# davidfang00/opticalflowdiffusion

Measured on NVIDIA B200. Metric: flows/sec DDIM-50 @436x1024, higher is better.
Workload: dtype bf16

## Files before the change

opticalflowdiffusion_b200/csrc/fd_conv_epi.cuh:

```cuda
#pragma once

#include "fd_tc.cuh"

namespace fdtc {

constexpr int kBlockM = 128;
constexpr int kEpiWarps = 8;
constexpr int kEpiThreads = kEpiWarps * 32;
constexpr int kSlabBytes = kBlockM * 128;

struct EpiTile {
  int img, h0, w0, n_tile;
};

struct EpiCtx {
  uint32_t tmem_base;
  uint32_t o_smem;
  uint32_t tfull0, tempty0;
  float* s_bias;
  float* s_stats;
  const CUtensorMap* map_out;
  const float* bias;
  const __nv_bfloat16* residual;
  double* gn_stats;
  int H, W, Cout, Wt;
  int shuffle_cq;
  float* head_out;
  const float* head_w;
  const float* head_b;
  int head_n, head_h0, head_w0, head_pt, head_pl;
  float* s_head;
  int phase;
  int dbg;
  int tempty_remote;
  const double* rt_stats;
  const float* rt_gamma;
  const float* rt_beta;
  float rt_eps;
  float* s_rt;
};

__device__ __forceinline__ float epi_silu_half(float h) {
  float t;
  asm("tanh.approx.f32 %0, %1;" : "=f"(t) : "f"(h));
  return fmaf(h, t, h);
}

__device__ __forceinline__ void mbar_arrive_cluster(uint32_t bar, uint32_t rank) {
  asm volatile(
      "{\n\t.reg .b32 ra;\n\t"
      "mapa.shared::cluster.u32 ra, %0, %1;\n\t"
      "mbarrier.arrive.shared::cluster.b64 _, [ra];\n\t}" ::"r"(bar),
      "r"(rank)
      : "memory");
}

template <int BLOCK_N, int GPT, int NBUF, int NACC = 2, class NextTile>
__device__ __forceinline__ void conv_epilogue(const EpiCtx& ec, NextTile next_tile) {
  constexpr int NCHUNK = BLOCK_N / 32;
  constexpr int CPW = NCHUNK / 2;
  constexpr int CPGT = GPT > 0 ? BLOCK_N / GPT : 32;
  constexpr int GIC = CPGT < 32 ? 32 / CPGT : 1;
  const int warp = threadIdx.x >> 5;
  const int lane = threadIdx.x & 31;
  const uint32_t tmem_base = ec.tmem_base;
  const uint32_t o_smem = ec.o_smem;
  float* const s_bias = ec.s_bias;
  float* const s_stats = ec.s_stats;
  {
    const int ew = warp - 2;
    const int et = threadIdx.x - 64;
    const int quarter = warp & 3;
    const int half = ew >> 2;
    const int row = quarter * 32 + lane;
    const int rr = row / ec.Wt, ww = row - rr * ec.Wt;
    float st_s[CPW > 0 ? CPW : 1][GIC], st_q[CPW > 0 ? CPW : 1][GIC];
#pragma unroll
    for (int a = 0; a < (CPW > 0 ? CPW : 1); ++a)
#pragma unroll
      for (int b = 0; b < GIC; ++b) st_s[a][b] = st_q[a][b] = 0.f;
    int st_img = -1, st_ntile = 0;
    int rt_img = -1, rt_ntile = -1;
    if (BLOCK_N == 64 && ec.head_out != nullptr) {
      for (int i = et; i < ec.head_n * 64; i += kEpiThreads) ec.s_head[i] = __ldg(ec.head_w + i);
    }
    uint32_t slab_count = 0;

    auto flush_stats = [&]() {
      if (GPT == 0 || st_img < 0) return;
      float* mine = s_stats + ew * 16;
      if (lane < 16) mine[lane] = 0.f;
      __syncwarp();
#pragma unroll
      for (int a = 0; a < (CPW > 0 ? CPW : 1); ++a)
#pragma unroll
        for (int b = 0; b < GIC; ++b) {
          const float s = fd_warp_sum(st_s[a][b]), q = fd_warp_sum(st_q[a][b]);
          if (lane == 0) {
            const int col = (2 * a + half) * 32 + b * CPGT;
            const int grp = col / CPGT;
            mine[grp * 2] += s;
            mine[grp * 2 + 1] += q;
          }
          st_s[a][b] = st_q[a][b] = 0.f;
        }
      named_bar_sync(2, kEpiThreads);
      if (et < 2 * GPT) {
        float sv = 0.f;
#pragma unroll
        for (int w8 = 0; w8 < kEpiWarps; ++w8) sv += s_stats[w8 * 16 + et];
        atomicAdd(ec.gn_stats + (long)st_img * 16 + st_ntile * 2 * GPT + et, (double)sv);
      }
      named_bar_sync(2, kEpiThreads);
    };

    EpiTile tc;
    for (int iter = 0; next_tile(iter, tc); ++iter) {
      const int as = iter % NACC;
      const uint32_t aphase = (iter / NACC) & 1;
      const int n_tile = tc.n_tile, img = tc.img, h0 = tc.h0, w0 = tc.w0;
      const int h = h0 + rr, w = w0 + ww;
      const bool valid = (h < ec.H) && (w < ec.W);
      const int n0 = n_tile * BLOCK_N;
      if (GPT > 0 && (img != st_img || n_tile != st_ntile)) {
        flush_stats();
        st_img = img;
        st_ntile = n_tile;
      }
      float* bias_s = s_bias + (as & 1) * BLOCK_N;
      for (int i = et; i < BLOCK_N; i += kEpiThreads) bias_s[i] = ec.bias ? __ldg(ec.bias + n0 + i) : 0.f;
      float* rt_s = ec.s_rt;
      if (ec.rt_stats != nullptr && (img != rt_img || n_tile != rt_ntile)) {
        rt_img = img;
        rt_ntile = n_tile;
        const int cpg = ec.Cout >> 3;
        const double cnt = (double)ec.H * (double)ec.W * (double)cpg;
        for (int i = et; i < BLOCK_N; i += kEpiThreads) {
          const int c = n0 + i;
          const int g = c / cpg;
          const double s = ec.rt_stats[((long)img * 8 + g) * 2], ss = ec.rt_stats[((long)img * 8 + g) * 2 + 1];
          const double mean = s / cnt;
          double var = ss / cnt - mean * mean;
          if (var < 0.0) var = 0.0;
          const float rstd = (float)(1.0 / sqrt(var + (double)ec.rt_eps));
          const float ga = __ldg(ec.rt_gamma + c) * rstd;
          rt_s[i] = 0.5f * ga;
          rt_s[BLOCK_N + i] = 0.5f * (__ldg(ec.rt_beta + c) - (float)mean * ga);
        }
      }

      const long pix = ((long)img * ec.H + h) * ec.W + w;
      const __nv_bfloat16* rrow = (ec.residual && valid) ? ec.residual + pix * ec.Cout + n0 : nullptr;
      uint4 rpre[4];
      if (rrow != nullptr) {
#pragma unroll
        for (int q = 0; q < 4; ++q) rpre[q] = __ldg(reinterpret_cast<const uint4*>(rrow + half * 32) + q);
      }
      mbar_wait(ec.tfull0 + 8u * as, aphase);
      tc_fence_after();
      if (ec.dbg & 8) {
        tc_fence_before();
        if (ec.tempty_remote) mbar_arrive_cluster(ec.tempty0 + 8u * as, 0);
        else mbar_arrive(ec.tempty0 + 8u * as);
        continue;
      }
#pragma unroll
      for (int slab = 0; slab < (BLOCK_N + 63) / 64; ++slab) {
        const uint32_t buf = o_smem + (slab_count % NBUF) * kSlabBytes;
        ++slab_count;
        if (ew == 0 && elect_one_sync()) tma_store_wait_read<NBUF - 1>();
        named_bar_sync(1, kEpiThreads);
        const int ci = slab * 2 + half;
        const int c = ci * 32;
        uint32_t acc[32];
        tmem_ld32(tmem_base + ((uint32_t)(quarter * 32) << 16) + (uint32_t)(as * BLOCK_N + c), acc);
        tmem_ld_wait();
        float v[32];
#pragma unroll
        for (int j4 = 0; j4 < 8; ++j4) {
          const float4 b4 = *reinterpret_cast<const float4*>(bias_s + c + j4 * 4);
          v[j4 * 4 + 0] = __uint_as_float(acc[j4 * 4 + 0]) + b4.x;
          v[j4 * 4 + 1] = __uint_as_float(acc[j4 * 4 + 1]) + b4.y;
          v[j4 * 4 + 2] = __uint_as_float(acc[j4 * 4 + 2]) + b4.z;
          v[j4 * 4 + 3] = __uint_as_float(acc[j4 * 4 + 3]) + b4.w;
        }
        if (rrow != nullptr) {
          uint4 rcur[4];
#pragma unroll
          for (int q = 0; q < 4; ++q) rcur[q] = rpre[q];
          if (slab + 1 < (BLOCK_N + 63) / 64) {
#pragma unroll
            for (int q = 0; q < 4; ++q) rpre[q] = __ldg(reinterpret_cast<const uint4*>(rrow + c + 64) + q);
          }
#pragma unroll
          for (int q = 0; q < 4; ++q) {
            const uint4 r4 = rcur[q];
            const uint32_t rw[4] = {r4.x, r4.y, r4.z, r4.w};
            if (ec.rt_stats != nullptr) {
              const float4 a0 = *reinterpret_cast<const float4*>(rt_s + c + q * 8), a1 = *reinterpret_cast<const float4*>(rt_s + c + q * 8 + 4);
              const float4 b0 = *reinterpret_cast<const float4*>(rt_s + BLOCK_N + c + q * 8),
                           b1 = *reinterpret_cast<const float4*>(rt_s + BLOCK_N + c + q * 8 + 4);
              const float aa[8] = {a0.x, a0.y, a0.z, a0.w, a1.x, a1.y, a1.z, a1.w};
              const float bb[8] = {b0.x, b0.y, b0.z, b0.w, b1.x, b1.y, b1.z, b1.w};
#pragma unroll
              for (int e = 0; e < 4; ++e) {
                const float2 f = fd_unpack_bf16(rw[e]);
                v[q * 8 + e * 2] += epi_silu_half(fmaf(aa[e * 2], f.x, bb[e * 2]));
                v[q * 8 + e * 2 + 1] += epi_silu_half(fmaf(aa[e * 2 + 1], f.y, bb[e * 2 + 1]));
              }
            } else {
#pragma unroll
              for (int e = 0; e < 4; ++e) {
                const float2 f = fd_unpack_bf16(rw[e]);
                v[q * 8 + e * 2] += f.x;
                v[q * 8 + e * 2 + 1] += f.y;
              }
            }
          }
        }
        if (GPT > 0 && valid) {
#pragma unroll
          for (int b = 0; b < GIC; ++b) {
            constexpr int span = CPGT < 32 ? CPGT : 32;
            float s = 0.f, q = 0.f;
#pragma unroll
            for (int j = 0; j < span; ++j) {
              const float x = v[b * span + j];
              s += x;
              q = fmaf(x, x, q);
            }
            st_s[slab][b] += s;
            st_q[slab][b] += q;
          }
        }
        if (BLOCK_N == 64 && ec.head_out != nullptr) {
          const float* hw = ec.s_head;
          float* hx = ec.s_head + 256 + (ew * 32 + lane) * 4;
          float d[4] = {0.f, 0.f, 0.f, 0.f};
#pragma unroll
          for (int o = 0; o < 4; ++o) {
            if (o < ec.head_n) {
#pragma unroll
              for (int j4 = 0; j4 < 8; ++j4) {
                const float4 w4 = *reinterpret_cast<const float4*>(hw + o * 64 + c + j4 * 4);
                d[o] = fmaf(v[j4 * 4 + 0], w4.x, d[o]);
                d[o] = fmaf(v[j4 * 4 + 1], w4.y, d[o]);
                d[o] = fmaf(v[j4 * 4 + 2], w4.z, d[o]);
                d[o] = fmaf(v[j4 * 4 + 3], w4.w, d[o]);
              }
            }
          }
          *reinterpret_cast<float4*>(hx) = make_float4(d[0], d[1], d[2], d[3]);
          tc_fence_before();
          if (ec.tempty_remote) mbar_arrive_cluster(ec.tempty0 + 8u * as, 0);
          else mbar_arrive(ec.tempty0 + 8u * as);
          named_bar_sync(1, kEpiThreads);
          if (half == 0 && valid) {
            const float4 o4 = *reinterpret_cast<const float4*>(ec.s_head + 256 + ((ew ^ 4) * 32 + lane) * 4);
            const float r4[4] = {d[0] + o4.x, d[1] + o4.y, d[2] + o4.z, d[3] + o4.w};
            const int hh = h - ec.head_pt, wq = w - ec.head_pl;
            if (hh >= 0 && hh < ec.head_h0 && wq >= 0 && wq < ec.head_w0) {
#pragma unroll
              for (int o = 0; o < 4; ++o)
                if (o < ec.head_n)
                  ec.head_out[(((long)img * ec.head_n + o) * ec.head_h0 + hh) * (long)ec.head_w0 + wq] = r4[o] + __ldg(ec.head_b + o);
            }
          }
          continue;
        }
        const uint32_t rbase = buf + (uint32_t)row * 128u;
#pragma unroll
        for (int q = 0; q < 4; ++q) {
          const uint32_t piece = (uint32_t)(half * 4 + q) ^ (uint32_t)(row & 7);
          const uint32_t o0 = fd_pack_bf16(v[q * 8 + 0], v[q * 8 + 1]), o1 = fd_pack_bf16(v[q * 8 + 2], v[q * 8 + 3]);
          const uint32_t o2 = fd_pack_bf16(v[q * 8 + 4], v[q * 8 + 5]), o3 = fd_pack_bf16(v[q * 8 + 6], v[q * 8 + 7]);
          asm volatile("st.shared.v4.b32 [%0], {%1, %2, %3, %4};" ::"r"(rbase + piece * 16u), "r"(o0), "r"(o1), "r"(o2),
                       "r"(o3)
                       : "memory");
        }
        fence_proxy_async_smem();
        if (slab == (BLOCK_N + 63) / 64 - 1) {
          tc_fence_before();
          if (ec.tempty_remote) mbar_arrive_cluster(ec.tempty0 + 8u * as, 0);
          else mbar_arrive(ec.tempty0 + 8u * as);
        }
        named_bar_sync(1, kEpiThreads);
        if (ew == 0 && elect_one_sync()) {
          const int cc = n0 + slab * 64;
          if (ec.shuffle_cq > 0) {
            const int pq = cc / ec.shuffle_cq;
            tma_store_5d(ec.map_out, buf, cc - pq * ec.shuffle_cq, pq & 1, w0, pq >> 1, h0);
          } else if (ec.phase >= 0) {
            tma_store_5d(ec.map_out, buf, cc, ec.phase & 1, w0, ec.phase >> 1, img * ec.H + h0);
          } else {
            tma_store_5d(ec.map_out, buf, cc, w0, h0, img, 0);
          }
          tma_store_commit();
        }
      }
    }
    flush_stats();
    __syncwarp();
    if (ew == 0 && elect_one_sync()) tma_store_wait_all();
  }
}

}
```

opticalflowdiffusion_b200/csrc/fd_conv_igemm.cu:

```cuda
#include "fd_conv_epi.cuh"

using namespace fdtc;

namespace {

constexpr int kBlockK = 64;
constexpr int kATileBytes = kBlockM * kBlockK * 2;
constexpr int kThreads = 64 + kEpiThreads + 32;

struct ConvParams {
  int N, H, W;
  int Cout;
  int KW;
  int taps;
  int pad_h, pad_w;
  int mode;
  int chunks0, chunks1;
  int R, Wt;
  int tiles_w, tiles_h, n_tiles, total_tiles;
  const float* bias;
  const __nv_bfloat16* residual;
  double* gn_stats;
  int shuffle_cq;
  int dbg;
  const double* rt_stats;
  const float* rt_gamma;
  const float* rt_beta;
  float rt_eps;
  int phase;
  float* head_out;
  const float* head_w;
  const float* head_b;
  int head_n, head_h0, head_w0, head_pt, head_pl;
};

template <int BLOCK_N, int SH = 0>
struct Cfg {
  static constexpr int kBTileBytes = BLOCK_N * kBlockK * 2;
  static constexpr int kStageBytes = kATileBytes + kBTileBytes;
  static constexpr int kStages = SH ? (BLOCK_N == 64 ? 6 : (BLOCK_N == 128 ? 5 : 3)) : (BLOCK_N == 64 ? 7 : (BLOCK_N == 128 ? 6 : 4));
  static constexpr int kStoreBufs = SH ? (BLOCK_N / 64 > 2 ? BLOCK_N / 64 : 2) : (BLOCK_N == 64 ? 2 : 1);
  static constexpr int kTmemCols = 2 * BLOCK_N;
  static constexpr int kHeadBytes = BLOCK_N == 64 ? (256 + kEpiWarps * 32 * 4) * 4 : 0;
  static constexpr int kTailBytes = 256  + 2 * BLOCK_N * 4  + kEpiWarps * 16 * 4  + 64 +
                                    4 * BLOCK_N * 4  + kHeadBytes;
  static constexpr int kSmemBytes = 1024 + kStages * kStageBytes + kStoreBufs * kSlabBytes + kTailBytes;
};

template <int BLOCK_N, int GPT, int SH>
__global__ void __launch_bounds__(kThreads, 1)
conv_igemm_kernel(const __grid_constant__ CUtensorMap map_a0, const __grid_constant__ CUtensorMap map_a1,
                  const __grid_constant__ CUtensorMap map_b, const __grid_constant__ CUtensorMap map_out,
                  const ConvParams p) {
  using C = Cfg<BLOCK_N, SH>;
  constexpr int STAGES = C::kStages;
  constexpr int NBUF = C::kStoreBufs;
  extern __shared__ uint8_t smem_raw[];
  const uint32_t base = (smem_u32(smem_raw) + 1023u) & ~1023u;
  uint8_t* gbase = smem_raw + (base - smem_u32(smem_raw));
  const uint32_t a_smem = base;
  const uint32_t b_smem = base + STAGES * kATileBytes;
  const uint32_t o_smem = base + STAGES * C::kStageBytes;
  const uint32_t bar_base = o_smem + NBUF * kSlabBytes;
  auto full_bar = [&](int s) { return bar_base + 8u * s; };
  auto empty_bar = [&](int s) { return bar_base + 8u * (STAGES + s); };
  auto tfull_bar = [&](int s) { return bar_base + 8u * (2 * STAGES + s); };
  auto tempty_bar = [&](int s) { return bar_base + 8u * (2 * STAGES + 2 + s); };
  uint8_t* gtail = gbase + STAGES * C::kStageBytes + NBUF * kSlabBytes + 256;
  float* s_bias = reinterpret_cast<float*>(gtail);
  float* s_stats = reinterpret_cast<float*>(gtail + 2 * BLOCK_N * 4);
  uint32_t* s_tmem = reinterpret_cast<uint32_t*>(gtail + 2 * BLOCK_N * 4 + kEpiWarps * 16 * 4);
  float* s_rt = reinterpret_cast<float*>(gtail + 2 * BLOCK_N * 4 + kEpiWarps * 16 * 4 + 64);
  float* s_head = s_rt + 4 * BLOCK_N;

  const int warp = threadIdx.x >> 5;
  const int lane = threadIdx.x & 31;
  const int cpt = p.chunks0 + p.chunks1;
  const int num_kb = p.taps * cpt;
  const int tiles_per_img = p.tiles_w * p.tiles_h;

  if (warp == 0 && lane == 0) {
    tma_prefetch_desc(&map_a0);
    tma_prefetch_desc(&map_a1);
    tma_prefetch_desc(&map_b);
    tma_prefetch_desc(&map_out);
    for (int s = 0; s < STAGES; ++s) {
      mbar_init(full_bar(s), 2);
      mbar_init(empty_bar(s), 1);
    }
    for (int s = 0; s < 2; ++s) {
      mbar_init(tfull_bar(s), 1);
      mbar_init(tempty_bar(s), kEpiThreads);
    }
    fence_barrier_init();
  }
  if (warp == 1) tmem_alloc(smem_u32(s_tmem), C::kTmemCols);
  tc_fence_before();
  __syncthreads();
  tc_fence_after();
  const uint32_t tmem_base = *s_tmem;

  if (warp == 0 || warp == 10) {
    if (elect_one_sync()) {
      int stage = opaque32(0);
      uint32_t phase = 0;
      const int tile0 = opaque32((int)blockIdx.x), tstep = opaque32((int)gridDim.x);
      if (warp == 0) {
        const bool skip = kDiag && (opaque32(p.dbg) & 1) != 0, mode0 = opaque32(p.mode) == 0;
        const int chunks0 = opaque32(p.chunks0), KW = opaque32(p.KW), cpt_ = opaque32(cpt), nkb = opaque32(num_kb);
        const uint64_t m0 = opaque64(reinterpret_cast<uint64_t>(&map_a0)), m1 = opaque64(reinterpret_cast<uint64_t>(&map_a1));
        for (int tile = tile0; tile < p.total_tiles; tile += tstep) {
          const int m_tile = tile / p.n_tiles;
          const int img = m_tile / tiles_per_img;
          const int rem = m_tile - img * tiles_per_img;
          const int th = rem / p.tiles_w;
          const int h0 = th * p.R;
          const int w0 = (rem - th * p.tiles_w) * p.Wt;
          const int bw = mode0 ? w0 - p.pad_w : 0, bh = mode0 ? h0 - p.pad_h : 0;
          int kx = 0, ky = 0, chunk = 0;
          for (int kb = 0; kb < nkb; ++kb) {
            const bool first = chunk < chunks0;
            const uint64_t ma = opaque64(first ? m0 : m1);
            const int c0 = opaque32((first ? chunk : chunk - chunks0) * kBlockK);
            const int c1 = opaque32(bw + kx);
            const int c2 = opaque32(mode0 ? bh + ky : w0);
            const int c3 = opaque32(mode0 ? img : ky);
            const int c4 = opaque32(mode0 ? 0 : h0);
            const uint32_t fb = (uint32_t)opaque32((int)full_bar(stage));
            const uint32_t dst = (uint32_t)opaque32((int)(a_smem + stage * kATileBytes));
            mbar_wait(empty_bar(stage), phase ^ 1u);
            if (skip) {
              mbar_arrive(fb);
            } else {
              mbar_expect_tx(fb, kATileBytes);
              tma_load_5d(dst, reinterpret_cast<const CUtensorMap*>(ma), fb, c0, c1, c2, c3, c4);
            }
            if (++stage == STAGES) { stage = 0; phase ^= 1u; }
            if (++chunk == cpt_) {
              chunk = 0;
              if (++kx == KW) { kx = 0; ++ky; }
            }
          }
        }
      } else {
        const bool skip = kDiag && (opaque32(p.dbg) & 2) != 0;
        const int nkb = opaque32(num_kb);
        const uint64_t mb = opaque64(reinterpret_cast<uint64_t>(&map_b));
        for (int tile = tile0; tile < p.total_tiles; tile += tstep) {
          const int n0 = (tile % p.n_tiles) * BLOCK_N;
          int k0 = 0;
          for (int kb = 0; kb < nkb; ++kb, k0 += kBlockK) {
            const uint32_t fb = (uint32_t)opaque32((int)full_bar(stage));
            const uint32_t dst = (uint32_t)opaque32((int)(b_smem + stage * C::kBTileBytes));
            const int ck = opaque32(k0), cn = opaque32(n0);
            mbar_wait(empty_bar(stage), phase ^ 1u);
            if (skip) {
              mbar_arrive(fb);
            } else {
              mbar_expect_tx(fb, C::kBTileBytes);
              tma_load_2d(dst, reinterpret_cast<const CUtensorMap*>(mb), fb, ck, cn);
            }
            if (++stage == STAGES) { stage = 0; phase ^= 1u; }
          }
        }
      }
    }
  } else if (warp == 1) {
    constexpr uint32_t idesc = umma_idesc_bf16(kBlockM, BLOCK_N);
    if (elect_one_sync()) {
      const uint64_t adesc0 = umma_desc_sw128(a_smem), bdesc0 = umma_desc_sw128(b_smem);
      int stage = 0;
      uint32_t phase = 0;
      int iter = 0;
      bool waited = false;
      const bool skip_mma = kDiag && (p.dbg & 4) != 0;
      uint64_t ad = opaque64(adesc0), bd = opaque64(bdesc0);
      for (int tile = blockIdx.x; tile < p.total_tiles; tile += gridDim.x, ++iter) {
        const int as = iter & 1;
        const uint32_t aphase = (iter >> 1) & 1;
        mbar_wait(tempty_bar(as), aphase ^ 1u);
        tc_fence_after();
        const uint32_t tmem_d = tmem_base + as * BLOCK_N;
        for (int kb = 0; kb < num_kb; ++kb) {
          if (!waited) mbar_wait(full_bar(stage), phase);
          tc_fence_after();
          if (!skip_mma) {
#pragma unroll
            for (int k = 0; k < kBlockK / 16; ++k) {
              umma_bf16(tmem_d, ad + (uint64_t)(2 * k), bd + (uint64_t)(2 * k), idesc, (kb | k) != 0 ? 1u : 0u);
            }
          }
          const uint32_t cur_empty = empty_bar(stage);
          if (++stage == STAGES) { stage = 0; phase ^= 1u; }
          ad = opaque64(adesc0 + (uint64_t)(stage * (kATileBytes >> 4)));
          bd = opaque64(bdesc0 + (uint64_t)(stage * (C::kBTileBytes >> 4)));
          waited = kb + 1 < num_kb;
          if (waited) mbar_wait(full_bar(stage), phase);
          umma_commit(cur_empty);
          if (kb == num_kb - 1) umma_commit(tfull_bar(as));
        }
      }
    }
    __syncwarp();
  } else if (warp >= 2 && warp < 2 + kEpiWarps) {
    EpiCtx ec;
    ec.tmem_base = tmem_base;
    ec.o_smem = o_smem;
    ec.tfull0 = tfull_bar(0);
    ec.tempty0 = tempty_bar(0);
    ec.s_bias = s_bias;
    ec.s_stats = s_stats;
    ec.map_out = &map_out;
    ec.bias = p.bias;
    ec.residual = p.residual;
    ec.gn_stats = p.gn_stats;
    ec.H = p.H; ec.W = p.W; ec.Cout = p.Cout; ec.Wt = p.Wt;
    ec.shuffle_cq = p.shuffle_cq;
    ec.tempty_remote = 0;
    ec.dbg = kDiag ? p.dbg : 0;
    ec.rt_stats = p.rt_stats; ec.rt_gamma = p.rt_gamma; ec.rt_beta = p.rt_beta; ec.rt_eps = p.rt_eps; ec.s_rt = s_rt;
    ec.phase = p.phase;
    ec.head_out = p.head_out; ec.head_w = p.head_w; ec.head_b = p.head_b; ec.head_n = p.head_n; ec.s_head = s_head;
    ec.head_h0 = p.head_h0; ec.head_w0 = p.head_w0; ec.head_pt = p.head_pt; ec.head_pl = p.head_pl;
    conv_epilogue<BLOCK_N, GPT, NBUF>(ec, [&](int iter, EpiTile& t) {
      const int tile = blockIdx.x + iter * gridDim.x;
      if (tile >= p.total_tiles) return false;
      t.n_tile = tile % p.n_tiles;
      const int m_tile = tile / p.n_tiles;
      t.img = m_tile / tiles_per_img;
      const int rem = m_tile - t.img * tiles_per_img;
      t.h0 = (rem / p.tiles_w) * p.R;
      t.w0 = (rem % p.tiles_w) * p.Wt;
      return true;
    });
  }

  tc_fence_before();
  __syncthreads();
  if (warp == 1) {
    tc_fence_after();
    tmem_dealloc(tmem_base, C::kTmemCols);
  }
}

constexpr uint32_t kPeerBitMask = 0xFEFFFFFFu;

__device__ __forceinline__ uint32_t cluster_ctarank() {
  uint32_t r;
  asm volatile("mov.u32 %0, %%cluster_ctarank;" : "=r"(r));
  return r;
}
__device__ __forceinline__ void cluster_sync_all() {
  asm volatile("barrier.cluster.arrive.release.aligned;" ::: "memory");
  asm volatile("barrier.cluster.wait.acquire.aligned;" ::: "memory");
}
__device__ __forceinline__ void tma2_load_5d(uint32_t dst, const CUtensorMap* m, uint32_t bar, int c0, int c1, int c2, int c3,
                                             int c4) {
  asm volatile(
      "cp.async.bulk.tensor.5d.cta_group::2.shared::cluster.global.mbarrier::complete_tx::bytes [%0], [%1, {%3, %4, %5, %6, %7}], [%2];" ::"r"(dst),
      "l"(m), "r"(bar & kPeerBitMask), "r"(c0), "r"(c1), "r"(c2), "r"(c3), "r"(c4)
      : "memory");
}
__device__ __forceinline__ void tma2_load_2d(uint32_t dst, const CUtensorMap* m, uint32_t bar, int c0, int c1) {
  asm volatile(
      "cp.async.bulk.tensor.2d.cta_group::2.shared::cluster.global.mbarrier::complete_tx::bytes [%0], [%1, {%3, %4}], [%2];" ::"r"(dst),
      "l"(m), "r"(bar & kPeerBitMask), "r"(c0), "r"(c1)
      : "memory");
}
__device__ __forceinline__ void umma2_bf16(uint32_t tmem_d, uint64_t adesc, uint64_t bdesc, uint32_t idesc, uint32_t accumulate) {
  asm volatile(
      "{\n\t.reg .pred p;\n\t"
      "setp.ne.b32 p, %4, 0;\n\t"
      "tcgen05.mma.cta_group::2.kind::f16 [%0], %1, %2, %3, p;\n\t}" ::"r"(tmem_d),
      "l"(adesc), "l"(bdesc), "r"(idesc), "r"(accumulate)
      : "memory");
}
__device__ __forceinline__ void umma2_commit(uint32_t bar) {
  asm volatile("tcgen05.commit.cta_group::2.mbarrier::arrive::one.shared::cluster.multicast::cluster.b64 [%0], %1;" ::"r"(bar),
               "h"((uint16_t)3)
               : "memory");
}

template <int BLOCK_N, int MT = 1>
struct PairCfg {
  static constexpr int kBHalfBytes = (BLOCK_N / 2) * kBlockK * 2;
  static constexpr int kStageBytes = MT * kATileBytes + kBHalfBytes;
  static constexpr int kStages = MT == 2 ? 5 : (BLOCK_N == 256 ? 5 : 7);
  static constexpr int kStoreBufs = MT == 2 ? 1 : 2;
  static constexpr int kAcc = 2 * MT;
  static constexpr int kTmemCols = kAcc * BLOCK_N;
  static constexpr int kTailBytes = 256 + 2 * BLOCK_N * 4 + kEpiWarps * 16 * 4 + 64 + 4 * BLOCK_N * 4;
  static constexpr int kSmemBytes = 1024 + kStages * kStageBytes + kStoreBufs * kSlabBytes + kTailBytes;
  static_assert(kTmemCols <= 512, "accumulators do not fit tensor memory");
};

template <int BLOCK_N, int GPT, int MT>
__global__ void __cluster_dims__(2, 1, 1) __launch_bounds__(kThreads, 1)
conv_igemm_pair_kernel(const __grid_constant__ CUtensorMap map_a0, const __grid_constant__ CUtensorMap map_a1,
                       const __grid_constant__ CUtensorMap map_b, const __grid_constant__ CUtensorMap map_out,
                       const ConvParams p) {
  using C = PairCfg<BLOCK_N, MT>;
  constexpr int STAGES = C::kStages;
  constexpr int NBUF = C::kStoreBufs;
  constexpr int NACC = C::kAcc;
  extern __shared__ uint8_t smem_raw[];
  const uint32_t base = (smem_u32(smem_raw) + 1023u) & ~1023u;
  uint8_t* gbase = smem_raw + (base - smem_u32(smem_raw));
  const uint32_t a_smem = base;
  const uint32_t b_smem = base + STAGES * MT * kATileBytes;
  const uint32_t o_smem = base + STAGES * C::kStageBytes;
  const uint32_t bar_base = o_smem + NBUF * kSlabBytes;
  auto full_bar = [&](int s) { return bar_base + 8u * s; };
  auto empty_bar = [&](int s) { return bar_base + 8u * (STAGES + s); };
  auto tfull_bar = [&](int s) { return bar_base + 8u * (2 * STAGES + s); };
  auto tempty_bar = [&](int s) { return bar_base + 8u * (2 * STAGES + NACC + s); };
  uint8_t* gtail = gbase + STAGES * C::kStageBytes + NBUF * kSlabBytes + 256;
  float* s_bias = reinterpret_cast<float*>(gtail);
  float* s_stats = reinterpret_cast<float*>(gtail + 2 * BLOCK_N * 4);
  uint32_t* s_tmem = reinterpret_cast<uint32_t*>(gtail + 2 * BLOCK_N * 4 + kEpiWarps * 16 * 4);
  float* s_rt = reinterpret_cast<float*>(gtail + 2 * BLOCK_N * 4 + kEpiWarps * 16 * 4 + 64);
  float* s_head = nullptr;

  const int warp = threadIdx.x >> 5;
  const int lane = threadIdx.x & 31;
  const uint32_t rank = cluster_ctarank();
  const int pair = blockIdx.x >> 1, npairs = gridDim.x >> 1;
  const int cpt = p.chunks0 + p.chunks1;
  const int num_kb = p.taps * cpt;
  const int tiles_per_img = p.tiles_w * p.tiles_h;
  const int super_tiles = p.total_tiles / (2 * MT);

  auto decode = [&](int st, int m, int& n_tile, int& img, int& h0, int& w0) {
    n_tile = st % p.n_tiles;
    const int m_tile = 2 * MT * (st / p.n_tiles) + (int)rank * MT + m;
    img = m_tile / tiles_per_img;
    const int rem = m_tile - img * tiles_per_img;
    h0 = (rem / p.tiles_w) * p.R;
    w0 = (rem % p.tiles_w) * p.Wt;
  };

  if (warp == 0 && lane == 0) {
    tma_prefetch_desc(&map_a0);
    tma_prefetch_desc(&map_a1);
    tma_prefetch_desc(&map_b);
    tma_prefetch_desc(&map_out);
    for (int s = 0; s < STAGES; ++s) {
      mbar_init(full_bar(s), 2);
      mbar_init(empty_bar(s), 1);
    }
    for (int s = 0; s < NACC; ++s) {
      mbar_init(tfull_bar(s), 1);
      mbar_init(tempty_bar(s), 2 * kEpiThreads);
    }
    fence_barrier_init();
  }
  if (warp == 1) {
    asm volatile("tcgen05.alloc.cta_group::2.sync.aligned.shared::cta.b32 [%0], %1;" ::"r"(smem_u32(s_tmem)), "r"(C::kTmemCols)
                 : "memory");
    asm volatile("tcgen05.relinquish_alloc_permit.cta_group::2.sync.aligned;" ::: "memory");
  }
  tc_fence_before();
  __syncthreads();
  cluster_sync_all();
  tc_fence_after();
  const uint32_t tmem_base = *s_tmem;

  if (warp == 0 || warp == 10) {
    if (elect_one_sync()) {
      int stage = opaque32(0);
      uint32_t phase = 0;
      const int st0 = opaque32(pair), ststep = opaque32(npairs), nkb = opaque32(num_kb);
      const bool leader = opaque32((int)rank) == 0;
      if (warp == 0) {
        const bool mode0 = opaque32(p.mode) == 0;
        const int chunks0 = opaque32(p.chunks0), KW = opaque32(p.KW), cpt_ = opaque32(cpt);
        const uint64_t m0 = opaque64(reinterpret_cast<uint64_t>(&map_a0)), m1 = opaque64(reinterpret_cast<uint64_t>(&map_a1));
        for (int st = st0; st < super_tiles; st += ststep) {
          int n_tile, img[MT], h0[MT], w0[MT], bw[MT], bh[MT];
#pragma unroll
          for (int m = 0; m < MT; ++m) {
            decode(st, m, n_tile, img[m], h0[m], w0[m]);
            bw[m] = mode0 ? w0[m] - p.pad_w : 0;
            bh[m] = mode0 ? h0[m] - p.pad_h : 0;
          }
          int kx = 0, ky = 0, chunk = 0;
          for (int kb = 0; kb < nkb; ++kb) {
            const bool first = chunk < chunks0;
            const uint64_t ma = opaque64(first ? m0 : m1);
            const int c0 = opaque32((first ? chunk : chunk - chunks0) * kBlockK);
            int c1[MT], c2[MT], c3[MT], c4[MT];
#pragma unroll
            for (int m = 0; m < MT; ++m) {
              c1[m] = opaque32(bw[m] + kx);
              c2[m] = opaque32(mode0 ? bh[m] + ky : w0[m]);
              c3[m] = opaque32(mode0 ? img[m] : ky);
              c4[m] = opaque32(mode0 ? 0 : h0[m]);
            }
            const uint32_t fb = (uint32_t)opaque32((int)full_bar(stage));
            const uint32_t dst = (uint32_t)opaque32((int)(a_smem + stage * MT * kATileBytes));
            mbar_wait(empty_bar(stage), phase ^ 1u);
            if (kDiag && (p.dbg & 1)) {
              if (leader) mbar_arrive(fb);
            } else {
              if (leader) mbar_expect_tx(fb, 2 * MT * kATileBytes);
#pragma unroll
              for (int m = 0; m < MT; ++m)
                tma2_load_5d(dst + m * kATileBytes, reinterpret_cast<const CUtensorMap*>(ma), fb, c0, c1[m], c2[m], c3[m], c4[m]);
            }
            if (++stage == STAGES) { stage = 0; phase ^= 1u; }
            if (++chunk == cpt_) {
              chunk = 0;
              if (++kx == KW) { kx = 0; ++ky; }
            }
          }
        }
      } else {
        const uint64_t mb = opaque64(reinterpret_cast<uint64_t>(&map_b));
        for (int st = st0; st < super_tiles; st += ststep) {
          const int n0 = (st % p.n_tiles) * BLOCK_N + (int)rank * (BLOCK_N / 2);
          int k0 = 0;
          for (int kb = 0; kb < nkb; ++kb, k0 += kBlockK) {
            const uint32_t fb = (uint32_t)opaque32((int)full_bar(stage));
            const uint32_t dst = (uint32_t)opaque32((int)(b_smem + stage * C::kBHalfBytes));
            const int ck = opaque32(k0), cn = opaque32(n0);
            mbar_wait(empty_bar(stage), phase ^ 1u);
            if (kDiag && (p.dbg & 2)) {
              if (leader) mbar_arrive(fb);
            } else {
              if (leader) mbar_expect_tx(fb, 2 * C::kBHalfBytes);
              tma2_load_2d(dst, reinterpret_cast<const CUtensorMap*>(mb), fb, ck, cn);
            }
            if (++stage == STAGES) { stage = 0; phase ^= 1u; }
          }
        }
      }
    }
  } else if (warp == 1) {
    if (rank == 0 && elect_one_sync()) {
      constexpr uint32_t idesc = umma_idesc_bf16(256, BLOCK_N);
      const uint64_t adesc0 = umma_desc_sw128(a_smem), bdesc0 = umma_desc_sw128(b_smem);
      int stage = 0;
      uint32_t phase = 0;
      int iter = 0;
      bool waited = false;
      uint64_t ad = opaque64(adesc0), bd = opaque64(bdesc0);
      for (int st = pair; st < super_tiles; st += npairs, ++iter) {
        const int as0 = (iter & 1) * MT;
        const uint32_t aphase = (iter >> 1) & 1;
#pragma unroll
        for (int m = 0; m < MT; ++m) mbar_wait(tempty_bar(as0 + m), aphase ^ 1u);
        tc_fence_after();
        const uint32_t tmem_d = tmem_base + as0 * BLOCK_N;
        for (int kb = 0; kb < num_kb; ++kb) {
          if (!waited) mbar_wait(full_bar(stage), phase);
          tc_fence_after();
#pragma unroll
          for (int m = 0; m < MT; ++m)
#pragma unroll
            for (int k = 0; k < kBlockK / 16; ++k)
              if (!(kDiag && (p.dbg & 4)))
                umma2_bf16(tmem_d + m * BLOCK_N, ad + (uint64_t)(m * (kATileBytes >> 4) + 2 * k), bd + (uint64_t)(2 * k), idesc,
                           (kb | k) != 0 ? 1u : 0u);
          const uint32_t cur_empty = empty_bar(stage);
          if (++stage == STAGES) { stage = 0; phase ^= 1u; }
          ad = opaque64(adesc0 + (uint64_t)(stage * (MT * kATileBytes >> 4)));
          bd = opaque64(bdesc0 + (uint64_t)(stage * (C::kBHalfBytes >> 4)));
          waited = kb + 1 < num_kb;
          if (waited) mbar_wait(full_bar(stage), phase);
          umma2_commit(cur_empty);
          if (kb == num_kb - 1) {
#pragma unroll
            for (int m = 0; m < MT; ++m) umma2_commit(tfull_bar(as0 + m));
          }
        }
      }
    }
    __syncwarp();
  } else if (warp >= 2 && warp < 2 + kEpiWarps) {
    EpiCtx ec;
    ec.tmem_base = tmem_base;
    ec.o_smem = o_smem;
    ec.tfull0 = tfull_bar(0);
    ec.tempty0 = tempty_bar(0);
    ec.s_bias = s_bias;
    ec.s_stats = s_stats;
    ec.map_out = &map_out;
    ec.bias = p.bias;
    ec.residual = p.residual;
    ec.gn_stats = p.gn_stats;
    ec.H = p.H; ec.W = p.W; ec.Cout = p.Cout; ec.Wt = p.Wt;
    ec.shuffle_cq = p.shuffle_cq;
    ec.tempty_remote = rank != 0;
    ec.dbg = kDiag ? p.dbg : 0;
    ec.rt_stats = p.rt_stats; ec.rt_gamma = p.rt_gamma; ec.rt_beta = p.rt_beta; ec.rt_eps = p.rt_eps; ec.s_rt = s_rt;
    ec.phase = p.phase;
    ec.head_out = p.head_out; ec.head_w = p.head_w; ec.head_b = p.head_b; ec.head_n = p.head_n; ec.s_head = s_head;
    ec.head_h0 = p.head_h0; ec.head_w0 = p.head_w0; ec.head_pt = p.head_pt; ec.head_pl = p.head_pl;
    conv_epilogue<BLOCK_N, GPT, NBUF, NACC>(ec, [&](int iter, EpiTile& t) {
      const int st = pair + (iter / MT) * npairs;
      if (st >= super_tiles) return false;
      decode(st, iter % MT, t.n_tile, t.img, t.h0, t.w0);
      return true;
    });
  }

  tc_fence_before();
  __syncthreads();
  cluster_sync_all();
  if (warp == 1) {
    tc_fence_after();
    asm volatile("tcgen05.dealloc.cta_group::2.sync.aligned.b32 %0, %1;" ::"r"(tmem_base), "r"(C::kTmemCols) : "memory");
  }
}

template <int BLOCK_N, int GPT, int MT = 1>
int launch_pair(const CUtensorMap& ma0, const CUtensorMap& ma1, const CUtensorMap& mb, const CUtensorMap& mo, const ConvParams& p,
                int sms, cudaStream_t st) {
  using C = PairCfg<BLOCK_N, MT>;
  static bool attr_set = false;
  if (!attr_set) {
    FD_CUDA(cudaFuncSetAttribute(conv_igemm_pair_kernel<BLOCK_N, GPT, MT>, cudaFuncAttributeMaxDynamicSharedMemorySize,
                                 C::kSmemBytes));
    attr_set = true;
  }
  const int units = p.total_tiles / MT;
  int grid = units < sms ? units : sms;
  grid &= ~1;
  conv_igemm_pair_kernel<BLOCK_N, GPT, MT><<<grid, kThreads, C::kSmemBytes, st>>>(ma0, ma1, mb, mo, p);
  FD_LAUNCH_CHECK();
  return FD_OK;
}

struct TileShape {
  int R, Wt;
};

TileShape pick_tile(int H, int W) {
  TileShape best{1, 128};
  long best_cost = -1;
  for (int wt = 128; wt >= 8; wt >>= 1) {
    const int r = 128 / wt;
    const long cost = (long)((W + wt - 1) / wt) * wt * (long)((H + r - 1) / r) * r;
    if (best_cost < 0 || cost < best_cost) {
      best_cost = cost;
      best = TileShape{r, wt};
    }
  }
  return best;
}

TileShape pick_tile_rows_divide(int H, int W) {
  TileShape best{1, 128};
  long best_cost = -1;
  for (int wt = 128; wt >= 8; wt >>= 1) {
    const int r = 128 / wt;
    if (H % r != 0) continue;
    const long cost = (long)((W + wt - 1) / wt) * wt * (long)H;
    if (best_cost < 0 || cost < best_cost) {
      best_cost = cost;
      best = TileShape{r, wt};
    }
  }
  return best;
}

template <int BLOCK_N, int GPT, int SH = 0>
int launch(const CUtensorMap& ma0, const CUtensorMap& ma1, const CUtensorMap& mb, const CUtensorMap& mo,
           const ConvParams& p, int sms, cudaStream_t st) {
  using C = Cfg<BLOCK_N, SH>;
  static bool attr_set = false;
  if (!attr_set) {
    FD_CUDA(cudaFuncSetAttribute(conv_igemm_kernel<BLOCK_N, GPT, SH>, cudaFuncAttributeMaxDynamicSharedMemorySize,
                                 C::kSmemBytes));
    attr_set = true;
  }
  const int grid = p.total_tiles < sms ? p.total_tiles : sms;
  conv_igemm_kernel<BLOCK_N, GPT, SH><<<grid, kThreads, C::kSmemBytes, st>>>(ma0, ma1, mb, mo, p);
  FD_LAUNCH_CHECK();
  return FD_OK;
}

}

int fd_conv3x3_strip_launch(const void* src0, int C0, const void* src1, int C1, const void* wpacked, const float* bias,
                            const void* residual,
                            void* out, double* gn_stats, int N, int H, int W, cudaStream_t st);

struct HeadArgs {
  float* out;
  const float* w;
  const float* b;
  int n, h0, w0, pt, pl;
};

static int conv_igemm_impl(const void* src0, int C0, const void* src1, int C1, const void* wpacked, const float* bias,
                           const void* residual, void* out, double* gn_stats, int N, int H, int W, int Cout, int KH, int KW,
                           int pad_h, int pad_w, int mode, int out_mode, const double* rt_stats, const float* rt_gamma,
                           const float* rt_beta, float rt_eps, void* stream, int phase = -1, const struct HeadArgs* head = nullptr);

extern "C" {

int fd_conv_igemm(const void* src0, int C0, const void* src1, int C1, const void* wpacked, const float* bias,
                  const void* residual, void* out, double* gn_stats, int N, int H, int W, int Cout, int KH, int KW,
                  int pad_h, int pad_w, int mode, void* stream) {
  return fd_conv_igemm_ex(src0, C0, src1, C1, wpacked, bias, residual, out, gn_stats, N, H, W, Cout, KH, KW, pad_h,
                          pad_w, mode, 0, stream);
}

int fd_conv_igemm_ex(const void* src0, int C0, const void* src1, int C1, const void* wpacked, const float* bias,
                     const void* residual, void* out, double* gn_stats, int N, int H, int W, int Cout, int KH, int KW,
                     int pad_h, int pad_w, int mode, int out_mode, void* stream) {
  return conv_igemm_impl(src0, C0, src1, C1, wpacked, bias, residual, out, gn_stats, N, H, W, Cout, KH, KW, pad_h, pad_w, mode,
                         out_mode, nullptr, nullptr, nullptr, 0.f, stream);
}

int fd_conv_igemm_rt(const void* src0, int C0, const void* src1, int C1, const void* wpacked, const float* bias,
                     const void* residual_raw, const double* res_stats, const float* res_gamma, const float* res_beta, float eps,
                     void* out, int N, int H, int W, int Cout, int KH, int KW, int pad_h, int pad_w, void* stream) {
  FD_REQUIRE(residual_raw && res_stats && res_gamma && res_beta, "conv_igemm_rt: null pointer");
  FD_REQUIRE(Cout % 64 == 0 && (Cout / 8) > 0, "conv_igemm_rt: Cout=%d", Cout);
  return conv_igemm_impl(src0, C0, src1, C1, wpacked, bias, residual_raw, out, nullptr, N, H, W, Cout, KH, KW, pad_h, pad_w, 0, 0,
                         res_stats, res_gamma, res_beta, eps, stream);
}

int fd_conv_igemm_rt_head(const void* src0, int C0, const void* src1, int C1, const void* wpacked, const float* bias,
                          const void* residual_raw, const double* res_stats, const float* res_gamma, const float* res_beta, float eps,
                          const float* head_w, const float* head_b, int head_n, float* out_nchw, int N, int H, int W, int H0, int W0,
                          int pad_top, int pad_left, void* stream) {
  FD_REQUIRE(residual_raw && res_stats && res_gamma && res_beta && head_w && head_b && out_nchw, "conv_igemm_rt_head: null pointer");
  FD_REQUIRE(head_n >= 1 && head_n <= 4, "conv_igemm_rt_head: head_n=%d (1..4)", head_n);
  FD_REQUIRE(H0 > 0 && W0 > 0 && pad_top >= 0 && pad_left >= 0 && pad_top + H0 <= H && pad_left + W0 <= W,
             "conv_igemm_rt_head: crop %dx%d at (%d, %d) outside %dx%d", H0, W0, pad_top, pad_left, H, W);
  const HeadArgs ha{out_nchw, head_w, head_b, head_n, H0, W0, pad_top, pad_left};
  return conv_igemm_impl(src0, C0, src1, C1, wpacked, bias, residual_raw, nullptr, nullptr, N, H, W, 64, 1, 1, 0, 0, 0, 0,
                         res_stats, res_gamma, res_beta, eps, stream, -1, &ha);
}

int fd_conv_igemm_up(const void* src, int Cin, const void* wpacked4, const float* bias, void* out, int N, int H, int W, int Cout,
                     void* stream) {
  FD_REQUIRE(src && wpacked4 && out, "conv_igemm_up: null pointer");
  FD_REQUIRE(Cin % 64 == 0 && Cout % 64 == 0, "conv_igemm_up: Cin=%d Cout=%d must be multiples of 64", Cin, Cout);
  const __nv_bfloat16* w4 = static_cast<const __nv_bfloat16*>(wpacked4);
  for (int ph = 0; ph < 4; ++ph) {
    const int a = ph >> 1, b = ph & 1;
    if (int e = conv_igemm_impl(src, Cin, nullptr, 0, w4 + (size_t)ph * Cout * 4 * Cin, bias, nullptr, out, nullptr, N, H, W, Cout, 2, 2,
                                1 - a, 1 - b, 0, 2, nullptr, nullptr, nullptr, 0.f, stream, ph))
      return e;
  }
  return FD_OK;
}

}

static int conv_igemm_impl(const void* src0, int C0, const void* src1, int C1, const void* wpacked, const float* bias,
                           const void* residual, void* out, double* gn_stats, int N, int H, int W, int Cout, int KH, int KW,
                           int pad_h, int pad_w, int mode, int out_mode, const double* rt_stats, const float* rt_gamma,
                           const float* rt_beta, float rt_eps, void* stream, int phase, const HeadArgs* head) {
  FD_REQUIRE(head == nullptr || (Cout == 64 && rt_stats != nullptr && out_mode == 0 && mode == 0 && gn_stats == nullptr && KH == 1 && KW == 1),
             "conv_igemm: the output head takes a 1x1 residual-transform conv with Cout = 64");
  if (head != nullptr && out == nullptr) out = const_cast<void*>(src0);
  FD_REQUIRE(out_mode == 0 || out_mode == 1 || out_mode == 2, "conv_igemm: out_mode %d", out_mode);
  FD_REQUIRE(out_mode != 2 || (mode == 0 && phase >= 0 && phase < 4 && residual == nullptr && gn_stats == nullptr && rt_stats == nullptr),
             "conv_igemm: the phase store takes a plain conv (no residual / statistics)");
  FD_REQUIRE(out_mode != 1 || (mode == 0 && KH == 1 && KW == 1 && pad_h == 0 && pad_w == 0 && C1 == 0 &&
                               residual == nullptr && gn_stats == nullptr && Cout % 256 == 0),
             "conv_igemm: the pixel-shuffle store is for 1x1 convs with Cout %% 256 == 0, no residual / statistics");
  FD_REQUIRE(src0 && wpacked && out, "conv_igemm: null pointer");
  FD_REQUIRE(N > 0 && H > 0 && W > 0, "conv_igemm: bad geometry N=%d H=%d W=%d", N, H, W);
  FD_REQUIRE(C0 > 0 && C0 % 64 == 0 && C1 >= 0 && C1 % 64 == 0, "conv_igemm: C0=%d C1=%d must be multiples of 64", C0, C1);
  FD_REQUIRE(src1 != nullptr || C1 == 0, "conv_igemm: C1 > 0 needs src1");
  FD_REQUIRE(Cout > 0 && Cout % 64 == 0, "conv_igemm: Cout=%d must be a multiple of 64", Cout);
  FD_REQUIRE(mode == 0 || mode == 1, "conv_igemm: mode %d", mode);
  FD_REQUIRE(mode == 0 || (C1 == 0 && gn_stats == nullptr), "conv_igemm: mode 1 takes one source and no statistics");
  FD_REQUIRE(KH >= 1 && KW >= 1 && KH * KW <= 64, "conv_igemm: bad kernel %dx%d", KH, KW);
  {
    const bool chans_ok = (C0 == 64 && (C1 == 0 || C1 == 64)) || (C0 == 128 && C1 == 0);
    if (mode == 0 && KH == 3 && KW == 3 && pad_h == 1 && pad_w == 1 && chans_ok && Cout == 64 && W >= 128 && out_mode == 0 &&
        rt_stats == nullptr)
      return fd_conv3x3_strip_launch(src0, C0, src1, C1, wpacked, bias, residual, out, gn_stats, N, H, W, (cudaStream_t)stream);
  }
  static int sms = 0;
  if (sms == 0) {
    int dev = 0;
    FD_CUDA(cudaGetDevice(&dev));
    FD_CUDA(cudaDeviceGetAttribute(&sms, cudaDevAttrMultiProcessorCount, dev));
  }
  ConvParams p{};
  p.Cout = Cout;
  p.mode = mode;
  p.chunks0 = C0 / 64;
  p.chunks1 = C1 / 64;
  p.bias = bias;
  p.residual = static_cast<const __nv_bfloat16*>(residual);
  p.gn_stats = gn_stats;
  p.rt_stats = rt_stats; p.rt_gamma = rt_gamma; p.rt_beta = rt_beta; p.rt_eps = rt_eps;
  p.phase = out_mode == 2 ? phase : -1;
  if (head != nullptr) {
    p.head_out = head->out; p.head_w = head->w; p.head_b = head->b; p.head_n = head->n;
    p.head_h0 = head->h0; p.head_w0 = head->w0; p.head_pt = head->pt; p.head_pl = head->pl;
  }
  CUtensorMap ma0, ma1, mb, mo;
  TileShape ts;
  if (mode == 0) {
    int n = N, h = H, w = W;
    if (out_mode == 1) {
      n = 1;
      h = N * H;
    } else if (KH == 1 && KW == 1 && pad_h == 0 && pad_w == 0 && gn_stats == nullptr && rt_stats == nullptr) {
      FD_REQUIRE((long)N * H * W < (1L << 31), "conv_igemm: too many pixels");
      w = N * H * W;
      h = 1;
      n = 1;
    }
    p.N = n; p.H = h; p.W = w;
    p.KW = KW;
    p.taps = KH * KW;
    p.pad_h = pad_h;
    p.pad_w = pad_w;
    ts = out_mode == 2 ? pick_tile_rows_divide(h, w) : pick_tile(h, w);
    const uint32_t box[5] = {64, (uint32_t)ts.Wt, (uint32_t)ts.R, 1, 1};
    {
      const uint64_t dims[5] = {(uint64_t)C0, (uint64_t)w, (uint64_t)h, (uint64_t)n, 1};
      const uint64_t str[4] = {(uint64_t)C0 * 2, (uint64_t)w * C0 * 2, (uint64_t)h * w * C0 * 2, (uint64_t)n * h * w * C0 * 2};
      if (int e = make_tmap_bf16(&ma0, src0, 5, dims, str, box)) return e;
    }
    if (C1 > 0) {
      const uint64_t dims[5] = {(uint64_t)C1, (uint64_t)w, (uint64_t)h, (uint64_t)n, 1};
      const uint64_t str[4] = {(uint64_t)C1 * 2, (uint64_t)w * C1 * 2, (uint64_t)h * w * C1 * 2, (uint64_t)n * h * w * C1 * 2};
      if (int e = make_tmap_bf16(&ma1, src1, 5, dims, str, box)) return e;
    } else {
      ma1 = ma0;
    }
  } else {
    p.N = 1; p.H = N * H; p.W = W;
    p.KW = 2;
    p.taps = 4;
    ts = pick_tile(p.H, p.W);
    const uint64_t dims[5] = {(uint64_t)C0, 2, (uint64_t)W, 2, (uint64_t)N * H};
    const uint64_t str[4] = {(uint64_t)C0 * 2, (uint64_t)2 * C0 * 2, (uint64_t)2 * W * C0 * 2, (uint64_t)4 * W * C0 * 2};
    const uint32_t box[5] = {64, 1, (uint32_t)ts.Wt, 1, (uint32_t)ts.R};
    if (int e = make_tmap_bf16(&ma0, src0, 5, dims, str, box)) return e;
    ma1 = ma0;
  }
  p.R = ts.R;
  p.Wt = ts.Wt;
  p.tiles_w = (p.W + ts.Wt - 1) / ts.Wt;
  p.tiles_h = (p.H + ts.R - 1) / ts.R;
  const int block_n = (Cout % 256 == 0) ? 256 : ((Cout % 128 == 0) ? 128 : 64);
  p.n_tiles = Cout / block_n;
  const long total = (long)p.N * p.tiles_w * p.tiles_h * p.n_tiles;
  FD_REQUIRE(total < (1L << 31), "conv_igemm: too many tiles");
  p.total_tiles = (int)total;
  const bool stats_ = gn_stats != nullptr;
  const bool store_heavy_ = !stats_ && p.taps * (p.chunks0 + p.chunks1) <= 4;
  static const int dbg = fd_diag_bits("FD_CONV_DBG");
  p.dbg = dbg;
  const bool use_pair = block_n >= 128 && !store_heavy_ && out_mode != 1 && ((long)p.N * p.tiles_w * p.tiles_h) % 2 == 0 &&
                        p.total_tiles >= 2;
  {
    const uint64_t K = (uint64_t)p.taps * (C0 + C1);
    const uint64_t dims[2] = {K, (uint64_t)Cout};
    const uint64_t str[1] = {K * 2};
    const uint32_t box[2] = {64, (uint32_t)(use_pair ? block_n / 2 : block_n)};
    if (int e = make_tmap_bf16(&mb, wpacked, 2, dims, str, box)) return e;
  }
  if (out_mode == 1) {
    const uint64_t cq = (uint64_t)Cout / 4;
    p.shuffle_cq = (int)cq;
    const uint64_t dims[5] = {cq, 2, (uint64_t)p.W, 2, (uint64_t)p.H};
    const uint64_t str[4] = {cq * 2, 2 * cq * 2, (uint64_t)2 * p.W * cq * 2, (uint64_t)4 * p.W * cq * 2};
    const uint32_t box[5] = {64, 1, (uint32_t)ts.Wt, 1, (uint32_t)ts.R};
    if (int e = make_tmap_bf16(&mo, out, 5, dims, str, box)) return e;
  } else if (out_mode == 2) {
    const uint64_t c = (uint64_t)Cout;
    const uint64_t dims[5] = {c, 2, (uint64_t)p.W, 2, (uint64_t)p.N * p.H};
    const uint64_t str[4] = {c * 2, 2 * c * 2, (uint64_t)2 * p.W * c * 2, (uint64_t)4 * p.W * c * 2};
    const uint32_t box[5] = {64, 1, (uint32_t)ts.Wt, 1, (uint32_t)ts.R};
    if (int e = make_tmap_bf16(&mo, out, 5, dims, str, box)) return e;
  } else {
    const uint64_t dims[5] = {(uint64_t)Cout, (uint64_t)p.W, (uint64_t)p.H, (uint64_t)p.N, 1};
    const uint64_t str[4] = {(uint64_t)Cout * 2, (uint64_t)p.W * Cout * 2, (uint64_t)p.H * p.W * Cout * 2,
                             (uint64_t)p.N * p.H * p.W * Cout * 2};
    const uint32_t box[5] = {64, (uint32_t)ts.Wt, (uint32_t)ts.R, 1, 1};
    if (int e = make_tmap_bf16(&mo, out, 5, dims, str, box)) return e;
  }
  cudaStream_t st = (cudaStream_t)stream;
  const bool stats = gn_stats != nullptr;
  if (stats) FD_REQUIRE(p.n_tiles == 1 || p.n_tiles == 2, "conv_igemm: statistics need Cout in {64,128,256,512}");
  const bool store_heavy = !stats && p.taps * (p.chunks0 + p.chunks1) <= 4;
  if (store_heavy) {
    if (block_n == 256) return launch<256, 0, 1>(ma0, ma1, mb, mo, p, sms, st);
    if (block_n == 128) return launch<128, 0, 1>(ma0, ma1, mb, mo, p, sms, st);
    return launch<64, 0, 1>(ma0, ma1, mb, mo, p, sms, st);
  }
  if (use_pair && block_n == 256) {
    if (!stats) return launch_pair<256, 0>(ma0, ma1, mb, mo, p, sms, st);
    return p.n_tiles == 1 ? launch_pair<256, 8>(ma0, ma1, mb, mo, p, sms, st) : launch_pair<256, 4>(ma0, ma1, mb, mo, p, sms, st);
  }
  if (use_pair) {
    const bool mt2 = ((long)p.N * p.tiles_w * p.tiles_h) % 4 == 0 && p.total_tiles >= 4;
    if (mt2) return stats ? launch_pair<128, 8, 2>(ma0, ma1, mb, mo, p, sms, st) : launch_pair<128, 0, 2>(ma0, ma1, mb, mo, p, sms, st);
    return stats ? launch_pair<128, 8>(ma0, ma1, mb, mo, p, sms, st) : launch_pair<128, 0>(ma0, ma1, mb, mo, p, sms, st);
  }
  if (block_n == 256) {
    if (!stats) return launch<256, 0>(ma0, ma1, mb, mo, p, sms, st);
    return p.n_tiles == 1 ? launch<256, 8>(ma0, ma1, mb, mo, p, sms, st) : launch<256, 4>(ma0, ma1, mb, mo, p, sms, st);
  }
  if (block_n == 128) return stats ? launch<128, 8>(ma0, ma1, mb, mo, p, sms, st) : launch<128, 0>(ma0, ma1, mb, mo, p, sms, st);
  return stats ? launch<64, 8>(ma0, ma1, mb, mo, p, sms, st) : launch<64, 0>(ma0, ma1, mb, mo, p, sms, st);
}
```

opticalflowdiffusion_b200/csrc/fd_conv_strip.cu:

```cuda
#include "fd_conv_epi.cuh"

using namespace fdtc;

namespace {

constexpr int kC = 64;
constexpr int kTileW = 128;
constexpr int kStripPx = kTileW + 2;
constexpr int kStripTx = kStripPx * 128;
constexpr int kStripBytes = 136 * 128;
constexpr int kNS = 5;
constexpr int kWTapBytes = kC * kC * 2;
constexpr int kWBytes = 9 * kWTapBytes;
constexpr int kThreads = 64 + kEpiThreads + 64;
constexpr int kTail = 256 + 2 * kC * 4 + kEpiWarps * 16 * 4 + 64;
constexpr int kSmemBytes = 1024 + kWBytes + kNS * kStripBytes + 2 * kSlabBytes + kTail;

__device__ __forceinline__ void utccp_128x256b(uint32_t tmem_dst, uint64_t sdesc) {
  asm volatile("tcgen05.cp.cta_group::1.128x256b [%0], %1;" ::"r"(tmem_dst), "l"(sdesc) : "memory");
}
__device__ __forceinline__ void umma_ts_bf16(uint32_t tmem_d, uint32_t tmem_a, uint64_t bdesc, uint32_t idesc, uint32_t accumulate) {
  asm volatile(
      "{\n\t.reg .pred p;\n\t"
      "setp.ne.b32 p, %4, 0;\n\t"
      "tcgen05.mma.cta_group::1.kind::f16 [%0], [%1], %2, %3, p;\n\t}" ::"r"(tmem_d),
      "r"(tmem_a), "l"(bdesc), "r"(idesc), "r"(accumulate)
      : "memory");
}
constexpr int kATmemCol0 = 2 * kC;
constexpr int kATmemSlotCols = 3 * (kC / 2);
constexpr int kATmemSlots = 4;

__device__ __forceinline__ float silu_tanh(float z) {
  const float h = 0.5f * z;
  float t;
  asm("tanh.approx.f32 %0, %1;" : "=f"(t) : "f"(h));
  return fmaf(h, t, h);
}

struct StripParams {
  int N, H, W;
  int wblocks, total_rows;
  int tile_w;
  int c_off;
  int w_k0, w_kstride;
  const float* bias;
  const __nv_bfloat16* residual;
  double* gn_stats;
  const double* in_stats;
  const float* in_gamma;
  const float* in_beta;
  const float* in_ss;
  long in_ss_stride;
  float in_eps;
  int dbg;
};

struct StripWalk {
  int cur, end;
  __device__ __forceinline__ explicit StripWalk(const StripParams& p) {
    cur = (int)((long)p.total_rows * blockIdx.x / gridDim.x);
    end = (int)((long)p.total_rows * (blockIdx.x + 1) / gridDim.x);
  }
  __device__ __forceinline__ bool next(const StripParams& p, int& n, int& w0, int& ra, int& rb) {
    if (cur >= end) return false;
    const int col = cur / p.H;
    ra = cur - col * p.H;
    const int rows = min(p.H - ra, end - cur);
    rb = ra + rows;
    n = col / p.wblocks;
    w0 = (col - n * p.wblocks) * p.tile_w;
    cur += rows;
    return true;
  }
};

template <int GPT, class NextTile>
__device__ __forceinline__ void strip_epilogue2(const EpiCtx& ec, NextTile next_tile) {
  const int warp = threadIdx.x >> 5, lane = threadIdx.x & 31;
  const int ew = warp - 2;
  const int quarter = warp & 3, group = ew >> 2;
  const int gt = (ew & 3) * 32 + lane;
  const int row = quarter * 32 + lane;
  const int bar_id = 1 + group;
  float* const bias_s = ec.s_bias + group * kC;
  float* const s_stats = ec.s_stats + group * 64;
  constexpr int NG = GPT > 0 ? GPT : 1;
  constexpr int CPG = kC / 8;
  float st_s[NG], st_q[NG];
#pragma unroll
  for (int b = 0; b < NG; ++b) st_s[b] = st_q[b] = 0.f;
  int st_img = -1;
  const uint32_t buf = ec.o_smem + group * kSlabBytes;
  if (gt < kC) bias_s[gt] = ec.bias ? __ldg(ec.bias + gt) : 0.f;
  named_bar_sync(bar_id, 128);

  auto flush_stats = [&]() {
    if (GPT == 0 || st_img < 0) return;
    float* mine = s_stats + (ew & 3) * 16;
#pragma unroll
    for (int b = 0; b < NG; ++b) {
      const float s = fd_warp_sum(st_s[b]), q = fd_warp_sum(st_q[b]);
      if (lane == 0) {
        mine[b * 2] = s;
        mine[b * 2 + 1] = q;
      }
      st_s[b] = st_q[b] = 0.f;
    }
    named_bar_sync(bar_id, 128);
    if (gt < 2 * GPT) {
      const float sv = (s_stats[gt] + s_stats[16 + gt]) + (s_stats[32 + gt] + s_stats[48 + gt]);
      atomicAdd(ec.gn_stats + (long)st_img * 16 + gt, (double)sv);
    }
    named_bar_sync(bar_id, 128);
  };

  EpiTile tc;
  for (int iter = 0; next_tile(iter, tc); ++iter) {
    if ((iter & 1) != group) continue;
    const int as = group;
    const uint32_t aphase = (iter >> 1) & 1;
    const int img = tc.img, h = tc.h0, w0 = tc.w0;
    const int w = w0 + row;
    const bool valid = w < ec.W;
    if (GPT > 0 && img != st_img) {
      flush_stats();
      st_img = img;
    }
    mbar_wait(ec.tfull0 + 8u * as, aphase);
    tc_fence_after();
    if (kDiag && (ec.dbg & 8)) {
      tc_fence_before();
      mbar_arrive(ec.tempty0 + 8u * as);
      continue;
    }
    uint32_t acc[2][32];
    const uint32_t taddr = ec.tmem_base + ((uint32_t)(quarter * 32) << 16) + (uint32_t)(as * kC);
    tmem_ld32(taddr, acc[0]);
    tmem_ld32(taddr + 32, acc[1]);
    tmem_ld_wait();
    tc_fence_before();
    mbar_arrive(ec.tempty0 + 8u * as);
    const long pix = ((long)img * ec.H + h) * ec.W + w;
    uint32_t packed[32];
#pragma unroll
    for (int hc = 0; hc < 2; ++hc) {
      float v[32];
#pragma unroll
      for (int j4 = 0; j4 < 8; ++j4) {
        const float4 b4 = *reinterpret_cast<const float4*>(bias_s + hc * 32 + j4 * 4);
        v[j4 * 4 + 0] = __uint_as_float(acc[hc][j4 * 4 + 0]) + b4.x;
        v[j4 * 4 + 1] = __uint_as_float(acc[hc][j4 * 4 + 1]) + b4.y;
        v[j4 * 4 + 2] = __uint_as_float(acc[hc][j4 * 4 + 2]) + b4.z;
        v[j4 * 4 + 3] = __uint_as_float(acc[hc][j4 * 4 + 3]) + b4.w;
      }
      if (ec.residual != nullptr && valid) {
        const __nv_bfloat16* rrow = ec.residual + pix * kC + hc * 32;
#pragma unroll
        for (int q = 0; q < 4; ++q) {
          const uint4 r4 = __ldg(reinterpret_cast<const uint4*>(rrow) + q);
          const uint32_t rw[4] = {r4.x, r4.y, r4.z, r4.w};
#pragma unroll
          for (int e = 0; e < 4; ++e) {
            const float2 f = fd_unpack_bf16(rw[e]);
            v[q * 8 + e * 2] += f.x;
            v[q * 8 + e * 2 + 1] += f.y;
          }
        }
      }
      if (GPT > 0 && valid) {
#pragma unroll
        for (int b = 0; b < 4; ++b) {
          float s = 0.f, q = 0.f;
#pragma unroll
          for (int j = 0; j < CPG; ++j) {
            const float x = v[b * CPG + j];
            s += x;
            q = fmaf(x, x, q);
          }
          st_s[(hc * 4 + b) % NG] += s;
          st_q[(hc * 4 + b) % NG] += q;
        }
      }
#pragma unroll
      for (int j = 0; j < 16; ++j) packed[hc * 16 + j] = fd_pack_bf16(v[2 * j], v[2 * j + 1]);
    }
    if ((ew & 3) == 0 && elect_one_sync()) tma_store_wait_read<0>();
    named_bar_sync(bar_id, 128);
    const uint32_t rbase = buf + (uint32_t)row * 128u;
#pragma unroll
    for (int q = 0; q < 8; ++q) {
      const uint32_t piece = (uint32_t)q ^ (uint32_t)(row & 7);
      asm volatile("st.shared.v4.b32 [%0], {%1, %2, %3, %4};" ::"r"(rbase + piece * 16u), "r"(packed[q * 4]),
                   "r"(packed[q * 4 + 1]), "r"(packed[q * 4 + 2]), "r"(packed[q * 4 + 3])
                   : "memory");
    }
    fence_proxy_async_smem();
    named_bar_sync(bar_id, 128);
    if ((ew & 3) == 0 && elect_one_sync()) {
      tma_store_5d(ec.map_out, buf, 0, w0, h, img, 0);
      tma_store_commit();
    }
  }
  flush_stats();
  __syncwarp();
  if ((ew & 3) == 0 && elect_one_sync()) tma_store_wait_all();
}

template <int GPT>
__global__ void __launch_bounds__(kThreads, 1)
conv3x3_strip_kernel(const __grid_constant__ CUtensorMap map_in, const __grid_constant__ CUtensorMap map_w,
                     const __grid_constant__ CUtensorMap map_out, const StripParams p) {
  extern __shared__ uint8_t smem_raw[];
  const uint32_t base = (smem_u32(smem_raw) + 1023u) & ~1023u;
  uint8_t* gbase = smem_raw + (base - smem_u32(smem_raw));
  const uint32_t w_smem = base;
  const uint32_t s_smem = base + kWBytes;
  const uint32_t o_smem = s_smem + kNS * kStripBytes;
  const uint32_t bar_base = o_smem + 2 * kSlabBytes;
  const uint32_t wfull_bar = bar_base;
  auto full_bar = [&](int s) { return bar_base + 8u * (1 + s); };
  auto empty_bar = [&](int s) { return bar_base + 8u * (1 + kNS + s); };
  auto tfull_bar = [&](int s) { return bar_base + 8u * (1 + 2 * kNS + s); };
  auto tempty_bar = [&](int s) { return bar_base + 8u * (3 + 2 * kNS + s); };
  auto xfull_bar = [&](int s) { return bar_base + 8u * (5 + 2 * kNS + s); };
  const bool fuse_in = p.in_stats != nullptr;
  uint8_t* gtail = gbase + kWBytes + kNS * kStripBytes + 2 * kSlabBytes + 256;
  float* s_bias = reinterpret_cast<float*>(gtail);
  float* s_stats = reinterpret_cast<float*>(gtail + 2 * kC * 4);
  uint32_t* s_tmem = reinterpret_cast<uint32_t*>(gtail + 2 * kC * 4 + kEpiWarps * 16 * 4);
  const int warp = threadIdx.x >> 5, lane = threadIdx.x & 31;

  if (warp == 0 && lane == 0) {
    tma_prefetch_desc(&map_in);
    tma_prefetch_desc(&map_w);
    tma_prefetch_desc(&map_out);
    mbar_init(wfull_bar, 1);
    for (int s = 0; s < kNS; ++s) {
      mbar_init(full_bar(s), 1);
      mbar_init(empty_bar(s), 1);
      mbar_init(xfull_bar(s), 64);
    }
    for (int s = 0; s < 2; ++s) {
      mbar_init(tfull_bar(s), 1);
      mbar_init(tempty_bar(s), 128);
    }
    fence_barrier_init();
  }
  constexpr uint32_t kTmemCols = 512;
  if (warp == 1) tmem_alloc(smem_u32(s_tmem), kTmemCols);
  tc_fence_before();
  __syncthreads();
  tc_fence_after();
  const uint32_t tmem_base = *s_tmem;

  if (warp == 0) {
    if (elect_one_sync()) {
      mbar_expect_tx(wfull_bar, kWBytes);
      for (int tap = 0; tap < 9; ++tap)
        tma_load_2d(w_smem + tap * kWTapBytes, &map_w, wfull_bar, tap * p.w_kstride + p.w_k0, 0);
      uint32_t seq = 0;
      StripWalk walk(p);
      int n, w0, ra, rb;
      while (walk.next(p, n, w0, ra, rb)) {
        for (int y = ra - 1; y <= rb; ++y, ++seq) {
          const int slot = seq % kNS;
          const uint32_t phase = (seq / kNS) & 1u;
          mbar_wait(empty_bar(slot), phase ^ 1u);
          mbar_expect_tx(full_bar(slot), kStripTx);
          tma_load_5d(s_smem + slot * kStripBytes, &map_in, full_bar(slot), p.c_off, w0 - 1, y, n, 0);
        }
      }
    }
  } else if (warp == 1) {
    if (elect_one_sync()) {
      constexpr uint32_t idesc = umma_idesc_bf16(kBlockM, kC);
      mbar_wait(wfull_bar, 0);
      tc_fence_after();
      const uint64_t bdesc0 = umma_desc_sw128(w_smem);
      const uint32_t a_tmem0 = tmem_base + kATmemCol0;
      StripWalk cwalk(p);
      int c_left = 0;
      uint32_t cseq = 0;
      auto ready_bar = [&](uint32_t slot) { return fuse_in ? xfull_bar(slot) : full_bar(slot); };
      auto copy_strip = [&]() {
        const uint32_t slot = cseq % kNS;
        mbar_wait(ready_bar(slot), (cseq / kNS) & 1u);
        tc_fence_after();
        const uint32_t dst = a_tmem0 + (cseq % kATmemSlots) * kATmemSlotCols;
        const uint64_t sd = umma_desc_sw128(s_smem + slot * kStripBytes);
#pragma unroll
        for (int kx = 0; kx < 3; ++kx)
#pragma unroll
          for (int k = 0; k < kC / 16; ++k)
            if (!(kDiag && (p.dbg & 64)))
            utccp_128x256b(dst + kx * (kC / 2) + k * 8, sd + (uint64_t)(kx * 8 + 2 * k));
        umma_commit(empty_bar(slot));
        ++cseq;
      };
      auto strips_left = [&]() {
        while (c_left == 0) {
          int cn, cw0, cra, crb;
          if (!cwalk.next(p, cn, cw0, cra, crb)) return false;
          c_left = crb - cra + 2;
        }
        return true;
      };
      struct Claim {
        bool more, inter;
        uint32_t slot, phase, dst;
        uint64_t sd;
      };
      auto claim = [&](uint32_t f) {
        Claim c{};
        c.more = cseq < f + 4 && strips_left();
        if (c.more) {
          c.slot = cseq % kNS;
          c.phase = (cseq / kNS) & 1u;
          c.dst = a_tmem0 + (cseq % kATmemSlots) * kATmemSlotCols;
          c.sd = umma_desc_sw128(s_smem + c.slot * kStripBytes);
          ++cseq;
          --c_left;
        }
        return c;
      };
      auto landed = [&](Claim& c) { c.inter = c.more && mbar_try_wait(ready_bar(c.slot), c.phase); };
      long long dg_t0 = 0, dg_mma = 0, dg_tail = 0;
      unsigned long long dg_ns0 = 0;
      if (kDiag) {
        dg_t0 = clock64();
        asm volatile("mov.u64 %0, %%globaltimer;" : "=l"(dg_ns0));
      }
      StripWalk walk(p);
      int wn, ww0, wra, wrb;
      int iter = 0;
      if (walk.next(p, wn, ww0, wra, wrb)) {
        int rows = wrb - wra, j = 0;
        uint32_t f = 0;
        while (cseq < f + 3) {
          strips_left();
          copy_strip();
          --c_left;
        }
        mbar_wait(tempty_bar(0), 1u);
        Claim cp = claim(f);
        landed(cp);
        tc_fence_after();
        while (true) {
          const int as = iter & 1;
          const uint32_t tmem_d = tmem_base + as * kC;
          bool has_next = false, boundary = false;
          uint32_t f_next = 0;
          Claim cp_next{};
          long long dg_m = 0;
          if (kDiag) dg_m = clock64();
#pragma unroll
          for (int ky = 0; ky < 3; ++ky) {
            const uint32_t a_strip = a_tmem0 + ((f + ky) % kATmemSlots) * kATmemSlotCols;
#pragma unroll
            for (int kx = 0; kx < 3; ++kx) {
              const uint64_t bdesc = bdesc0 + (uint64_t)((ky * 3 + kx) * (kWTapBytes >> 4));
#pragma unroll
              for (int k = 0; k < kC / 16; ++k) {
                if (!(kDiag && (p.dbg & 4)))
                  umma_ts_bf16(tmem_d, a_strip + kx * (kC / 2) + k * 8, bdesc + (uint64_t)(2 * k), idesc, (ky | kx | k) != 0 ? 1u : 0u);
                const int m = (ky * 3 + kx) * 4 + k;
                if (m % 3 == 2 && cp.inter && !(kDiag && (p.dbg & 64))) {
                  const int c = m / 3, ckx = c >> 2, ck = c & 3;
                  utccp_128x256b(cp.dst + ckx * (kC / 2) + ck * 8, cp.sd + (uint64_t)(ckx * 8 + 2 * ck));
                }
                if (m == 5) {
                  if (j + 1 < rows) {
                    has_next = true;
                    f_next = f + 1;
                  } else if (walk.next(p, wn, ww0, wra, wrb)) {
                    has_next = boundary = true;
                    f_next = f + 3;
                  }
                }
                if (m == 14 && has_next && !boundary) cp_next = claim(f_next);
                if (m == 23 && has_next && !boundary) mbar_wait(tempty_bar((iter + 1) & 1), (((iter + 1) >> 1) & 1) ^ 1u);
                if (m == 32 && has_next && !boundary) landed(cp_next);
              }
            }
          }
          umma_commit(tfull_bar(as));
          if (kDiag) { dg_mma += clock64() - dg_m; dg_m = clock64(); }
          if (cp.inter) {
            umma_commit(empty_bar(cp.slot));
          } else if (cp.more) {
            mbar_wait(ready_bar(cp.slot), cp.phase);
            tc_fence_after();
#pragma unroll
            for (int c = 0; c < 12; ++c)
              if (!(kDiag && (p.dbg & 64))) utccp_128x256b(cp.dst + (c >> 2) * (kC / 2) + (c & 3) * 8, cp.sd + (uint64_t)((c >> 2) * 8 + 2 * (c & 3)));
            umma_commit(empty_bar(cp.slot));
          }
          if (!has_next) break;
          if (boundary) {
            rows = wrb - wra;
            j = 0;
            while (cseq < f_next + 3) {
              strips_left();
              copy_strip();
              --c_left;
            }
            mbar_wait(tempty_bar((iter + 1) & 1), (((iter + 1) >> 1) & 1) ^ 1u);
            cp_next = claim(f_next);
            landed(cp_next);
          } else {
            ++j;
          }
          tc_fence_after();
          f = f_next;
          cp = cp_next;
          ++iter;
          if (kDiag) dg_tail += clock64() - dg_m;
        }
        ++iter;
      }
      if (kDiag && (p.dbg & 128) && (blockIdx.x == 0 || blockIdx.x == 77)) {
        unsigned long long ns1;
        asm volatile("mov.u64 %0, %%globaltimer;" : "=l"(ns1));
        const long long cyc = clock64() - dg_t0;
        printf("strip TS issuer block %d: %d tiles, %lld cycles (%.0f / tile): MMA stream %lld, between tiles %lld, %llu ns -> %.2f GHz\n",
               blockIdx.x, iter, cyc, (double)cyc / iter, dg_mma, dg_tail, ns1 - dg_ns0, (double)cyc / (double)(ns1 - dg_ns0));
      }
    }
    __syncwarp();
  } else if (warp == 10 || warp == 11) {
    if (fuse_in) {
      const int tl = (warp - 10) * 32 + lane;
      const int q = tl & 7, r0 = tl >> 3;
      float a[8], b[8];
      int cur_n = -1;
      uint32_t seq = 0;
      StripWalk walk(p);
      int n, w0, ra, rb;
      while (walk.next(p, n, w0, ra, rb)) {
        if (n != cur_n) {
          cur_n = n;
          const int C = kC, cpg = C >> 3;
          const double cnt = (double)p.H * (double)p.W * cpg;
          const int g = (q * 8) / cpg;
          const double sm = p.in_stats[((long)n * 8 + g) * 2], ss = p.in_stats[((long)n * 8 + g) * 2 + 1];
          const double mean = sm / cnt;
          double var = ss / cnt - mean * mean;
          if (var < 0.0) var = 0.0;
          const float rstd = (float)(1.0 / sqrt(var + (double)p.in_eps));
#pragma unroll
          for (int j = 0; j < 8; ++j) {
            const int c = q * 8 + j;
            float ga = __ldg(p.in_gamma + c) * rstd;
            float be = __ldg(p.in_beta + c) - (float)mean * ga;
            if (p.in_ss != nullptr) {
              const float sc = __ldg(p.in_ss + (long)n * p.in_ss_stride + c) + 1.f;
              const float sh = __ldg(p.in_ss + (long)n * p.in_ss_stride + C + c);
              ga *= sc;
              be = be * sc + sh;
            }
            a[j] = 0.5f * ga;
            b[j] = 0.5f * be;
          }
        }
        for (int y = ra - 1; y <= rb; ++y, ++seq) {
          const uint32_t slot = seq % kNS;
          mbar_wait(full_bar(slot), (seq / kNS) & 1u);
          if (y >= 0 && y < p.H) {
            const int rlo = w0 > 0 ? 0 : 1 - w0;
            const int rhi = min(kStripPx, p.W - w0 + 1);
            int r = r0 < rlo ? r0 + (((rlo - r0) + 7) & ~7) : r0;
            uint8_t* gp8 = gbase + kWBytes + slot * kStripBytes + r * 128 + ((q ^ r0) << 4);
#pragma unroll 4
            for (; r < rhi; r += 8, gp8 += 1024) {
              uint4* gp = reinterpret_cast<uint4*>(gp8);
              const uint4 v = *gp;
              const uint32_t xw[4] = {v.x, v.y, v.z, v.w};
              float o[8];
#pragma unroll
              for (int e = 0; e < 4; ++e) {
                const float h0 = fmaf(a[2 * e], __uint_as_float(xw[e] << 16), b[2 * e]);
                const float h1 = fmaf(a[2 * e + 1], __uint_as_float(xw[e] & 0xffff0000u), b[2 * e + 1]);
                float t0, t1;
                asm("tanh.approx.f32 %0, %1;" : "=f"(t0) : "f"(h0));
                asm("tanh.approx.f32 %0, %1;" : "=f"(t1) : "f"(h1));
                o[2 * e] = fmaf(h0, t0, h0);
                o[2 * e + 1] = fmaf(h1, t1, h1);
              }
              uint4 w4;
              w4.x = fd_pack_bf16(o[0], o[1]);
              w4.y = fd_pack_bf16(o[2], o[3]);
              w4.z = fd_pack_bf16(o[4], o[5]);
              w4.w = fd_pack_bf16(o[6], o[7]);
              *gp = w4;
            }
          }
          fence_proxy_async_smem();
          mbar_arrive(xfull_bar(slot));
        }
      }
    }
  } else if (warp >= 2 && warp < 2 + kEpiWarps) {
    EpiCtx ec;
    ec.tmem_base = tmem_base;
    ec.o_smem = o_smem;
    ec.tfull0 = tfull_bar(0);
    ec.tempty0 = tempty_bar(0);
    ec.s_bias = s_bias;
    ec.s_stats = s_stats;
    ec.map_out = &map_out;
    ec.bias = p.bias;
    ec.residual = p.residual;
    ec.gn_stats = p.gn_stats;
    ec.H = p.H; ec.W = p.W; ec.Cout = kC; ec.Wt = kTileW;
    ec.shuffle_cq = 0;
    ec.tempty_remote = 0;
    ec.dbg = kDiag ? p.dbg : 0;
    ec.rt_stats = nullptr; ec.rt_gamma = nullptr; ec.rt_beta = nullptr; ec.rt_eps = 0.f; ec.s_rt = nullptr;
    ec.phase = -1;
    ec.head_out = nullptr; ec.head_w = nullptr; ec.head_b = nullptr; ec.head_n = 0; ec.s_head = nullptr;
    ec.head_h0 = ec.head_w0 = ec.head_pt = ec.head_pl = 0;
    StripWalk walk(p);
    int j = 0, n = 0, w0 = 0, ra = 0, rb = 0;
    auto next = [&](int, EpiTile& t) {
      while (ra + j >= rb) {
        if (!walk.next(p, n, w0, ra, rb)) return false;
        j = 0;
      }
      t.img = n;
      t.h0 = ra + j;
      t.w0 = w0;
      t.n_tile = 0;
      ++j;
      return true;
    };
    strip_epilogue2<GPT>(ec, next);
  }

  tc_fence_before();
  __syncthreads();
  if (warp == 1) {
    tc_fence_after();
    tmem_dealloc(tmem_base, kTmemCols);
  }
}

}

struct StripInputNorm {
  const double* stats;
  const float *gamma, *beta, *scale_shift;
  long ss_stride;
  float eps;
};

static int strip_launch(const void* src0, int C0, const void* src1, int C1, const void* wpacked, const float* bias,
                        const void* residual, void* out, double* gn_stats, int N, int H, int W, const StripInputNorm& in,
                        cudaStream_t st);

int fd_conv3x3_strip_launch(const void* src0, int C0, const void* src1, int C1, const void* wpacked, const float* bias,
                            const void* residual, void* out, double* gn_stats, int N, int H, int W, cudaStream_t st) {
  return strip_launch(src0, C0, src1, C1, wpacked, bias, residual, out, gn_stats, N, H, W, StripInputNorm{}, st);
}

extern "C" int fd_conv3x3_gnsilu_in(const void* src, const double* in_stats, const float* in_gamma, const float* in_beta,
                                    const float* in_scale_shift, long in_ss_stride, float in_eps, const void* wpacked,
                                    const float* bias, const void* residual, void* out, double* gn_stats, int N, int H, int W,
                                    void* stream) {
  FD_REQUIRE(src && in_stats && in_gamma && in_beta && wpacked && out && N > 0 && H > 0 && W >= 64,
             "conv3x3_gnsilu_in: bad argument (needs 64 -> 64 channels, W >= 64)");
  StripInputNorm in{in_stats, in_gamma, in_beta, in_scale_shift, in_ss_stride, in_eps};
  return strip_launch(src, 64, nullptr, 0, wpacked, bias, residual, out, gn_stats, N, H, W, in, (cudaStream_t)stream);
}

static int strip_launch(const void* src0, int C0, const void* src1, int C1, const void* wpacked, const float* bias,
                        const void* residual, void* out, double* gn_stats, int N, int H, int W, const StripInputNorm& in,
                        cudaStream_t st) {
  static int sms = 0;
  if (sms == 0) {
    int dev = 0;
    FD_CUDA(cudaGetDevice(&dev));
    FD_CUDA(cudaDeviceGetAttribute(&sms, cudaDevAttrMultiProcessorCount, dev));
  }
  const int cin = C0 + C1;
  const int passes = cin / 64;
  StripParams p{};
  p.N = N; p.H = H; p.W = W;
  p.tile_w = kTileW;
  p.wblocks = (W + p.tile_w - 1) / p.tile_w;
  p.total_rows = N * p.wblocks * H;
  p.w_kstride = cin;
  CUtensorMap mw, mo;
  {
    const uint64_t dO[5] = {(uint64_t)kC, (uint64_t)W, (uint64_t)H, (uint64_t)N, 1};
    const uint64_t sO[4] = {(uint64_t)kC * 2, (uint64_t)W * kC * 2, (uint64_t)H * W * kC * 2, (uint64_t)N * H * W * kC * 2};
    const uint32_t box_out[5] = {64, (uint32_t)p.tile_w, 1, 1, 1};
    if (int e = make_tmap_bf16(&mo, out, 5, dO, sO, box_out)) return e;
    const uint64_t K = (uint64_t)9 * cin;
    const uint64_t dims[2] = {K, (uint64_t)kC};
    const uint64_t str[1] = {K * 2};
    const uint32_t box[2] = {64, 64};
    if (int e = make_tmap_bf16(&mw, wpacked, 2, dims, str, box)) return e;
  }
  const int grid = p.total_rows < sms ? p.total_rows : sms;
  static bool attr_set = false;
  if (!attr_set) {
    FD_CUDA(cudaFuncSetAttribute(conv3x3_strip_kernel<8>, cudaFuncAttributeMaxDynamicSharedMemorySize, kSmemBytes));
    FD_CUDA(cudaFuncSetAttribute(conv3x3_strip_kernel<0>, cudaFuncAttributeMaxDynamicSharedMemorySize, kSmemBytes));
    attr_set = true;
  }
  p.in_stats = in.stats;
  p.in_gamma = in.gamma;
  p.in_beta = in.beta;
  p.in_ss = in.scale_shift;
  p.in_ss_stride = in.ss_stride;
  p.in_eps = in.eps;
  static const int dbg = fd_diag_bits("FD_CONV_DBG");
  p.dbg = dbg;
  for (int pass = 0; pass < passes; ++pass) {
    const bool last = pass == passes - 1;
    const bool from1 = pass == 1 && C1 > 0;
    const void* src = from1 ? src1 : src0;
    const int csrc = from1 ? C1 : C0;
    CUtensorMap mi;
    const uint64_t d[5] = {(uint64_t)csrc, (uint64_t)W, (uint64_t)H, (uint64_t)N, 1};
    const uint64_t sB[4] = {(uint64_t)csrc * 2, (uint64_t)W * csrc * 2, (uint64_t)H * W * csrc * 2, (uint64_t)N * H * W * csrc * 2};
    const uint32_t box_in[5] = {64, (uint32_t)kStripPx, 1, 1, 1};
    if (int e = make_tmap_bf16(&mi, src, 5, d, sB, box_in)) return e;
    p.c_off = (pass == 1 && C1 == 0) ? 64 : 0;
    p.w_k0 = pass * 64;
    p.bias = last ? bias : nullptr;
    p.residual = static_cast<const __nv_bfloat16*>(pass > 0 ? out : residual);
    p.gn_stats = last ? gn_stats : nullptr;
    if (p.gn_stats != nullptr) conv3x3_strip_kernel<8><<<grid, kThreads, kSmemBytes, st>>>(mi, mw, mo, p);
    else conv3x3_strip_kernel<0><<<grid, kThreads, kSmemBytes, st>>>(mi, mw, mo, p);
    FD_LAUNCH_CHECK();
  }
  return FD_OK;
}
```

Baseline: 9.216.

## Prefetch conv residual tiles into a shared-memory ring via TMA

Residual tensors added in the conv epilogues were previously read per thread with __ldg (with a one-slab register prefetch). They are now loaded by TMA into a small mbarrier-guarded shared-memory ring that is issued ahead across tiles, in both the igemm/pair kernels and the strip conv kernel. The aim is to take global residual latency off the epilogue's critical path. Bias reloads are also skipped when the n-tile is unchanged, and the head bias is cached in shared memory. The cost is extra shared memory, which drops one pipeline stage for some configs, plus more barriers and more complexity.

```diff
diff --git a/opticalflowdiffusion_b200/csrc/fd_conv_epi.cuh b/opticalflowdiffusion_b200/csrc/fd_conv_epi.cuh
--- a/opticalflowdiffusion_b200/csrc/fd_conv_epi.cuh
+++ b/opticalflowdiffusion_b200/csrc/fd_conv_epi.cuh
@@ -22,6 +22,9 @@
   const CUtensorMap* map_out;
   const float* bias;
   const __nv_bfloat16* residual;
+  const CUtensorMap* map_res;
+  uint32_t r_smem;
+  uint32_t rfull0;
   double* gn_stats;
   int H, W, Cout, Wt;
   int shuffle_cq;
@@ -55,8 +58,11 @@
       : "memory");
 }
 
-template <int BLOCK_N, int GPT, int NBUF, int NACC = 2, class NextTile>
+template <int BLOCK_N, int GPT, int NBUF, int NACC = 2, int RS = 0, class NextTile>
 __device__ __forceinline__ void conv_epilogue(const EpiCtx& ec, NextTile next_tile) {
+  static_assert(RS == 0 || RS >= 2, "a one-slot residual ring is no deeper than the register prefetch");
+  constexpr int NSLAB = (BLOCK_N + 63) / 64;
+  constexpr uint32_t kRS = RS > 0 ? RS : 1;
   constexpr int NCHUNK = BLOCK_N / 32;
   constexpr int CPW = NCHUNK / 2;
   constexpr int CPGT = GPT > 0 ? BLOCK_N / GPT : 32;
@@ -81,10 +87,24 @@
       for (int b = 0; b < GIC; ++b) st_s[a][b] = st_q[a][b] = 0.f;
     int st_img = -1, st_ntile = 0;
     int rt_img = -1, rt_ntile = -1;
+    int bias_nt0 = -1, bias_nt1 = -1;
     if (BLOCK_N == 64 && ec.head_out != nullptr) {
       for (int i = et; i < ec.head_n * 64; i += kEpiThreads) ec.s_head[i] = __ldg(ec.head_w + i);
+      if (et < ec.head_n) ec.s_head[256 + kEpiThreads * 4 + et] = __ldg(ec.head_b + et);
     }
     uint32_t slab_count = 0;
+    const bool rtma = RS > 0 && ec.residual != nullptr;
+    auto res_issue = [&](uint32_t s) {
+      EpiTile t;
+      if (!next_tile((int)(s / NSLAB), t)) return;
+      const uint32_t slot = s % kRS;
+      const uint32_t bar = ec.rfull0 + 8u * slot;
+      mbar_expect_tx(bar, kSlabBytes);
+      tma_load_5d(ec.r_smem + slot * kSlabBytes, ec.map_res, bar, t.n_tile * BLOCK_N + (int)(s % NSLAB) * 64, t.w0, t.h0,
+                  t.img, 0);
+    };
+    if (rtma && ew == 0 && elect_one_sync())
+      for (int s = 0; s < RS; ++s) res_issue((uint32_t)s);
 
     auto flush_stats = [&]() {
       if (GPT == 0 || st_img < 0) return;
@@ -128,7 +148,11 @@
         st_ntile = n_tile;
       }
       float* bias_s = s_bias + (as & 1) * BLOCK_N;
-      for (int i = et; i < BLOCK_N; i += kEpiThreads) bias_s[i] = ec.bias ? __ldg(ec.bias + n0 + i) : 0.f;
+      if (((as & 1) ? bias_nt1 : bias_nt0) != n_tile) {
+        if (as & 1) bias_nt1 = n_tile;
+        else bias_nt0 = n_tile;
+        for (int i = et; i < BLOCK_N; i += kEpiThreads) bias_s[i] = ec.bias ? __ldg(ec.bias + n0 + i) : 0.f;
+      }
       float* rt_s = ec.s_rt;
       if (ec.rt_stats != nullptr && (img != rt_img || n_tile != rt_ntile)) {
         rt_img = img;
@@ -150,7 +174,7 @@
       }
 
       const long pix = ((long)img * ec.H + h) * ec.W + w;
-      const __nv_bfloat16* rrow = (ec.residual && valid) ? ec.residual + pix * ec.Cout + n0 : nullptr;
+      const __nv_bfloat16* rrow = (RS == 0 && ec.residual && valid) ? ec.residual + pix * ec.Cout + n0 : nullptr;
       uint4 rpre[4];
       if (rrow != nullptr) {
 #pragma unroll
@@ -162,10 +186,20 @@
         tc_fence_before();
         if (ec.tempty_remote) mbar_arrive_cluster(ec.tempty0 + 8u * as, 0);
         else mbar_arrive(ec.tempty0 + 8u * as);
+        if (rtma) {
+          for (int slab = 0; slab < NSLAB; ++slab, ++slab_count) {
+            if (ew == 0 && elect_one_sync()) {
+              mbar_wait(ec.rfull0 + 8u * (slab_count % kRS), (slab_count / kRS) & 1u);
+              res_issue(slab_count + RS);
+            }
+            __syncwarp();
+          }
+        }
         continue;
       }
 #pragma unroll
-      for (int slab = 0; slab < (BLOCK_N + 63) / 64; ++slab) {
+      for (int slab = 0; slab < NSLAB; ++slab) {
+        const uint32_t rs_seq = slab_count;
         const uint32_t buf = o_smem + (slab_count % NBUF) * kSlabBytes;
         ++slab_count;
         if (ew == 0 && elect_one_sync()) tma_store_wait_read<NBUF - 1>();
@@ -184,14 +218,33 @@
           v[j4 * 4 + 2] = __uint_as_float(acc[j4 * 4 + 2]) + b4.z;
           v[j4 * 4 + 3] = __uint_as_float(acc[j4 * 4 + 3]) + b4.w;
         }
-        if (rrow != nullptr) {
-          uint4 rcur[4];
+        uint4 rcur[4];
+        bool radd = false;
+        if (RS > 0) {
+          if (rtma) {
+            const uint32_t slot = rs_seq % kRS;
+            mbar_wait(ec.rfull0 + 8u * slot, (rs_seq / kRS) & 1u);
+            radd = valid;
+            const uint32_t rb = ec.r_smem + slot * kSlabBytes + (uint32_t)row * 128u;
+#pragma unroll
+            for (int q = 0; q < 4; ++q) {
+              const uint32_t piece = (uint32_t)(half * 4 + q) ^ (uint32_t)(row & 7);
+              asm volatile("ld.shared.v4.b32 {%0, %1, %2, %3}, [%4];"
+                           : "=r"(rcur[q].x), "=r"(rcur[q].y), "=r"(rcur[q].z), "=r"(rcur[q].w)
+                           : "r"(rb + piece * 16u)
+                           : "memory");
+            }
+          }
+        } else if (rrow != nullptr) {
+          radd = true;
 #pragma unroll
           for (int q = 0; q < 4; ++q) rcur[q] = rpre[q];
-          if (slab + 1 < (BLOCK_N + 63) / 64) {
+          if (slab + 1 < NSLAB) {
 #pragma unroll
             for (int q = 0; q < 4; ++q) rpre[q] = __ldg(reinterpret_cast<const uint4*>(rrow + c + 64) + q);
           }
+        }
+        if (radd) {
 #pragma unroll
           for (int q = 0; q < 4; ++q) {
             const uint4 r4 = rcur[q];
@@ -255,6 +308,8 @@
           if (ec.tempty_remote) mbar_arrive_cluster(ec.tempty0 + 8u * as, 0);
           else mbar_arrive(ec.tempty0 + 8u * as);
           named_bar_sync(1, kEpiThreads);
+          if (rtma && ew == 0 && elect_one_sync()) res_issue(rs_seq + RS);
+          __syncwarp();
           if (half == 0 && valid) {
             const float4 o4 = *reinterpret_cast<const float4*>(ec.s_head + 256 + ((ew ^ 4) * 32 + lane) * 4);
             const float r4[4] = {d[0] + o4.x, d[1] + o4.y, d[2] + o4.z, d[3] + o4.w};
@@ -263,7 +318,7 @@
 #pragma unroll
               for (int o = 0; o < 4; ++o)
                 if (o < ec.head_n)
-                  ec.head_out[(((long)img * ec.head_n + o) * ec.head_h0 + hh) * (long)ec.head_w0 + wq] = r4[o] + __ldg(ec.head_b + o);
+                  ec.head_out[(((long)img * ec.head_n + o) * ec.head_h0 + hh) * (long)ec.head_w0 + wq] = r4[o] + ec.s_head[256 + kEpiThreads * 4 + o];
             }
           }
           continue;
@@ -286,6 +341,7 @@
         }
         named_bar_sync(1, kEpiThreads);
         if (ew == 0 && elect_one_sync()) {
+          if (rtma) res_issue(rs_seq + RS);
           const int cc = n0 + slab * 64;
           if (ec.shuffle_cq > 0) {
             const int pq = cc / ec.shuffle_cq;
diff --git a/opticalflowdiffusion_b200/csrc/fd_conv_igemm.cu b/opticalflowdiffusion_b200/csrc/fd_conv_igemm.cu
--- a/opticalflowdiffusion_b200/csrc/fd_conv_igemm.cu
+++ b/opticalflowdiffusion_b200/csrc/fd_conv_igemm.cu
@@ -34,39 +34,46 @@
   int head_n, head_h0, head_w0, head_pt, head_pl;
 };
 
-template <int BLOCK_N, int SH = 0>
+template <int BLOCK_N, int SH = 0, int RES = 0>
 struct Cfg {
+  static_assert(!RES || (SH && BLOCK_N <= 128), "residual ring: store-heavy N = 64 / 128 tiles only");
   static constexpr int kBTileBytes = BLOCK_N * kBlockK * 2;
   static constexpr int kStageBytes = kATileBytes + kBTileBytes;
-  static constexpr int kStages = SH ? (BLOCK_N == 64 ? 6 : (BLOCK_N == 128 ? 5 : 3)) : (BLOCK_N == 64 ? 7 : (BLOCK_N == 128 ? 6 : 4));
+  static constexpr int kStages = SH ? (BLOCK_N == 64 ? 6 : (BLOCK_N == 128 ? (RES ? 4 : 5) : 3)) : (BLOCK_N == 64 ? 7 : (BLOCK_N == 128 ? 6 : 4));
   static constexpr int kStoreBufs = SH ? (BLOCK_N / 64 > 2 ? BLOCK_N / 64 : 2) : (BLOCK_N == 64 ? 2 : 1);
+  static constexpr int kResBufs = RES ? (BLOCK_N == 64 ? 2 : 3) : 0;
   static constexpr int kTmemCols = 2 * BLOCK_N;
-  static constexpr int kHeadBytes = BLOCK_N == 64 ? (256 + kEpiWarps * 32 * 4) * 4 : 0;
+  static constexpr int kHeadBytes = BLOCK_N == 64 ? (256 + kEpiWarps * 32 * 4 + 4) * 4 : 0;
   static constexpr int kTailBytes = 256  + 2 * BLOCK_N * 4  + kEpiWarps * 16 * 4  + 64 +
                                     4 * BLOCK_N * 4  + kHeadBytes;
-  static constexpr int kSmemBytes = 1024 + kStages * kStageBytes + kStoreBufs * kSlabBytes + kTailBytes;
+  static constexpr int kSmemBytes = 1024 + kStages * kStageBytes + (kStoreBufs + kResBufs) * kSlabBytes + kTailBytes;
+  static_assert(kSmemBytes <= 232448, "shared memory");
+  static_assert(2 * kStages + 4 + kResBufs <= 32, "barriers");
 };
 
-template <int BLOCK_N, int GPT, int SH>
+template <int BLOCK_N, int GPT, int SH, int RES>
 __global__ void __launch_bounds__(kThreads, 1)
 conv_igemm_kernel(const __grid_constant__ CUtensorMap map_a0, const __grid_constant__ CUtensorMap map_a1,
                   const __grid_constant__ CUtensorMap map_b, const __grid_constant__ CUtensorMap map_out,
-                  const ConvParams p) {
-  using C = Cfg<BLOCK_N, SH>;
+                  const __grid_constant__ CUtensorMap map_res, const ConvParams p) {
+  using C = Cfg<BLOCK_N, SH, RES>;
   constexpr int STAGES = C::kStages;
   constexpr int NBUF = C::kStoreBufs;
+  constexpr int RS = C::kResBufs;
   extern __shared__ uint8_t smem_raw[];
   const uint32_t base = (smem_u32(smem_raw) + 1023u) & ~1023u;
   uint8_t* gbase = smem_raw + (base - smem_u32(smem_raw));
   const uint32_t a_smem = base;
   const uint32_t b_smem = base + STAGES * kATileBytes;
   const uint32_t o_smem = base + STAGES * C::kStageBytes;
-  const uint32_t bar_base = o_smem + NBUF * kSlabBytes;
+  const uint32_t r_smem = o_smem + NBUF * kSlabBytes;
+  const uint32_t bar_base = r_smem + RS * kSlabBytes;
   auto full_bar = [&](int s) { return bar_base + 8u * s; };
   auto empty_bar = [&](int s) { return bar_base + 8u * (STAGES + s); };
   auto tfull_bar = [&](int s) { return bar_base + 8u * (2 * STAGES + s); };
   auto tempty_bar = [&](int s) { return bar_base + 8u * (2 * STAGES + 2 + s); };
-  uint8_t* gtail = gbase + STAGES * C::kStageBytes + NBUF * kSlabBytes + 256;
+  auto rfull_bar = [&](int s) { return bar_base + 8u * (2 * STAGES + 4 + s); };
+  uint8_t* gtail = gbase + STAGES * C::kStageBytes + (NBUF + RS) * kSlabBytes + 256;
   float* s_bias = reinterpret_cast<float*>(gtail);
   float* s_stats = reinterpret_cast<float*>(gtail + 2 * BLOCK_N * 4);
   uint32_t* s_tmem = reinterpret_cast<uint32_t*>(gtail + 2 * BLOCK_N * 4 + kEpiWarps * 16 * 4);
@@ -84,6 +91,7 @@
     tma_prefetch_desc(&map_a1);
     tma_prefetch_desc(&map_b);
     tma_prefetch_desc(&map_out);
+    if (RS > 0 && p.residual != nullptr) tma_prefetch_desc(&map_res);
     for (int s = 0; s < STAGES; ++s) {
       mbar_init(full_bar(s), 2);
       mbar_init(empty_bar(s), 1);
@@ -92,6 +100,7 @@
       mbar_init(tfull_bar(s), 1);
       mbar_init(tempty_bar(s), kEpiThreads);
     }
+    for (int s = 0; s < RS; ++s) mbar_init(rfull_bar(s), 1);
     fence_barrier_init();
   }
   if (warp == 1) tmem_alloc(smem_u32(s_tmem), C::kTmemCols);
@@ -213,6 +222,9 @@
     ec.map_out = &map_out;
     ec.bias = p.bias;
     ec.residual = p.residual;
+    ec.map_res = &map_res;
+    ec.r_smem = r_smem;
+    ec.rfull0 = rfull_bar(0);
     ec.gn_stats = p.gn_stats;
     ec.H = p.H; ec.W = p.W; ec.Cout = p.Cout; ec.Wt = p.Wt;
     ec.shuffle_cq = p.shuffle_cq;
@@ -222,7 +234,7 @@
     ec.phase = p.phase;
     ec.head_out = p.head_out; ec.head_w = p.head_w; ec.head_b = p.head_b; ec.head_n = p.head_n; ec.s_head = s_head;
     ec.head_h0 = p.head_h0; ec.head_w0 = p.head_w0; ec.head_pt = p.head_pt; ec.head_pl = p.head_pl;
-    conv_epilogue<BLOCK_N, GPT, NBUF>(ec, [&](int iter, EpiTile& t) {
+    conv_epilogue<BLOCK_N, GPT, NBUF, 2, RS>(ec, [&](int iter, EpiTile& t) {
       const int tile = blockIdx.x + iter * gridDim.x;
       if (tile >= p.total_tiles) return false;
       t.n_tile = tile % p.n_tiles;
@@ -281,40 +293,47 @@
                : "memory");
 }
 
-template <int BLOCK_N, int MT = 1>
+template <int BLOCK_N, int MT = 1, int RES = 0>
 struct PairCfg {
+  static_assert(!RES || (BLOCK_N == 256 && MT == 1), "residual ring: N = 256 pairs only");
   static constexpr int kBHalfBytes = (BLOCK_N / 2) * kBlockK * 2;
   static constexpr int kStageBytes = MT * kATileBytes + kBHalfBytes;
-  static constexpr int kStages = MT == 2 ? 5 : (BLOCK_N == 256 ? 5 : 7);
+  static constexpr int kStages = MT == 2 ? 5 : (BLOCK_N == 256 ? (RES ? 4 : 5) : 7);
   static constexpr int kStoreBufs = MT == 2 ? 1 : 2;
+  static constexpr int kResBufs = RES ? 3 : 0;
   static constexpr int kAcc = 2 * MT;
   static constexpr int kTmemCols = kAcc * BLOCK_N;
   static constexpr int kTailBytes = 256 + 2 * BLOCK_N * 4 + kEpiWarps * 16 * 4 + 64 + 4 * BLOCK_N * 4;
-  static constexpr int kSmemBytes = 1024 + kStages * kStageBytes + kStoreBufs * kSlabBytes + kTailBytes;
+  static constexpr int kSmemBytes = 1024 + kStages * kStageBytes + (kStoreBufs + kResBufs) * kSlabBytes + kTailBytes;
   static_assert(kTmemCols <= 512, "accumulators do not fit tensor memory");
+  static_assert(kSmemBytes <= 232448, "shared memory");
+  static_assert(2 * kStages + 2 * kAcc + kResBufs <= 32, "barriers");
 };
 
-template <int BLOCK_N, int GPT, int MT>
+template <int BLOCK_N, int GPT, int MT, int RES>
 __global__ void __cluster_dims__(2, 1, 1) __launch_bounds__(kThreads, 1)
 conv_igemm_pair_kernel(const __grid_constant__ CUtensorMap map_a0, const __grid_constant__ CUtensorMap map_a1,
                        const __grid_constant__ CUtensorMap map_b, const __grid_constant__ CUtensorMap map_out,
-                       const ConvParams p) {
-  using C = PairCfg<BLOCK_N, MT>;
+                       const __grid_constant__ CUtensorMap map_res, const ConvParams p) {
+  using C = PairCfg<BLOCK_N, MT, RES>;
   constexpr int STAGES = C::kStages;
   constexpr int NBUF = C::kStoreBufs;
   constexpr int NACC = C::kAcc;
+  constexpr int RS = C::kResBufs;
   extern __shared__ uint8_t smem_raw[];
   const uint32_t base = (smem_u32(smem_raw) + 1023u) & ~1023u;
   uint8_t* gbase = smem_raw + (base - smem_u32(smem_raw));
   const uint32_t a_smem = base;
   const uint32_t b_smem = base + STAGES * MT * kATileBytes;
   const uint32_t o_smem = base + STAGES * C::kStageBytes;
-  const uint32_t bar_base = o_smem + NBUF * kSlabBytes;
+  const uint32_t r_smem = o_smem + NBUF * kSlabBytes;
+  const uint32_t bar_base = r_smem + RS * kSlabBytes;
   auto full_bar = [&](int s) { return bar_base + 8u * s; };
   auto empty_bar = [&](int s) { return bar_base + 8u * (STAGES + s); };
   auto tfull_bar = [&](int s) { return bar_base + 8u * (2 * STAGES + s); };
   auto tempty_bar = [&](int s) { return bar_base + 8u * (2 * STAGES + NACC + s); };
-  uint8_t* gtail = gbase + STAGES * C::kStageBytes + NBUF * kSlabBytes + 256;
+  auto rfull_bar = [&](int s) { return bar_base + 8u * (2 * STAGES + 2 * NACC + s); };
+  uint8_t* gtail = gbase + STAGES * C::kStageBytes + (NBUF + RS) * kSlabBytes + 256;
   float* s_bias = reinterpret_cast<float*>(gtail);
   float* s_stats = reinterpret_cast<float*>(gtail + 2 * BLOCK_N * 4);
   uint32_t* s_tmem = reinterpret_cast<uint32_t*>(gtail + 2 * BLOCK_N * 4 + kEpiWarps * 16 * 4);
@@ -352,6 +371,8 @@
       mbar_init(tfull_bar(s), 1);
       mbar_init(tempty_bar(s), 2 * kEpiThreads);
     }
+    for (int s = 0; s < RS; ++s) mbar_init(rfull_bar(s), 1);
+    if (RS > 0 && p.residual != nullptr) tma_prefetch_desc(&map_res);
     fence_barrier_init();
   }
   if (warp == 1) {
@@ -487,6 +508,7 @@
     ec.map_out = &map_out;
     ec.bias = p.bias;
     ec.residual = p.residual;
+    ec.map_res = &map_res; ec.r_smem = r_smem; ec.rfull0 = rfull_bar(0);
     ec.gn_stats = p.gn_stats;
     ec.H = p.H; ec.W = p.W; ec.Cout = p.Cout; ec.Wt = p.Wt;
     ec.shuffle_cq = p.shuffle_cq;
@@ -496,7 +518,7 @@
     ec.phase = p.phase;
     ec.head_out = p.head_out; ec.head_w = p.head_w; ec.head_b = p.head_b; ec.head_n = p.head_n; ec.s_head = s_head;
     ec.head_h0 = p.head_h0; ec.head_w0 = p.head_w0; ec.head_pt = p.head_pt; ec.head_pl = p.head_pl;
-    conv_epilogue<BLOCK_N, GPT, NBUF, NACC>(ec, [&](int iter, EpiTile& t) {
+    conv_epilogue<BLOCK_N, GPT, NBUF, NACC, RS>(ec, [&](int iter, EpiTile& t) {
       const int st = pair + (iter / MT) * npairs;
       if (st >= super_tiles) return false;
       decode(st, iter % MT, t.n_tile, t.img, t.h0, t.w0);
@@ -513,20 +535,20 @@
   }
 }
 
-template <int BLOCK_N, int GPT, int MT = 1>
-int launch_pair(const CUtensorMap& ma0, const CUtensorMap& ma1, const CUtensorMap& mb, const CUtensorMap& mo, const ConvParams& p,
-                int sms, cudaStream_t st) {
-  using C = PairCfg<BLOCK_N, MT>;
+template <int BLOCK_N, int GPT, int MT = 1, int RES = 0>
+int launch_pair(const CUtensorMap& ma0, const CUtensorMap& ma1, const CUtensorMap& mb, const CUtensorMap& mo, const CUtensorMap& mr,
+                const ConvParams& p, int sms, cudaStream_t st) {
+  using C = PairCfg<BLOCK_N, MT, RES>;
   static bool attr_set = false;
   if (!attr_set) {
-    FD_CUDA(cudaFuncSetAttribute(conv_igemm_pair_kernel<BLOCK_N, GPT, MT>, cudaFuncAttributeMaxDynamicSharedMemorySize,
+    FD_CUDA(cudaFuncSetAttribute(conv_igemm_pair_kernel<BLOCK_N, GPT, MT, RES>, cudaFuncAttributeMaxDynamicSharedMemorySize,
                                  C::kSmemBytes));
     attr_set = true;
   }
   const int units = p.total_tiles / MT;
   int grid = units < sms ? units : sms;
   grid &= ~1;
-  conv_igemm_pair_kernel<BLOCK_N, GPT, MT><<<grid, kThreads, C::kSmemBytes, st>>>(ma0, ma1, mb, mo, p);
+  conv_igemm_pair_kernel<BLOCK_N, GPT, MT, RES><<<grid, kThreads, C::kSmemBytes, st>>>(ma0, ma1, mb, mo, mr, p);
   FD_LAUNCH_CHECK();
   return FD_OK;
 }
@@ -564,18 +586,18 @@
   return best;
 }
 
-template <int BLOCK_N, int GPT, int SH = 0>
-int launch(const CUtensorMap& ma0, const CUtensorMap& ma1, const CUtensorMap& mb, const CUtensorMap& mo,
+template <int BLOCK_N, int GPT, int SH = 0, int RES = 0>
+int launch(const CUtensorMap& ma0, const CUtensorMap& ma1, const CUtensorMap& mb, const CUtensorMap& mo, const CUtensorMap& mr,
            const ConvParams& p, int sms, cudaStream_t st) {
-  using C = Cfg<BLOCK_N, SH>;
+  using C = Cfg<BLOCK_N, SH, RES>;
   static bool attr_set = false;
   if (!attr_set) {
-    FD_CUDA(cudaFuncSetAttribute(conv_igemm_kernel<BLOCK_N, GPT, SH>, cudaFuncAttributeMaxDynamicSharedMemorySize,
+    FD_CUDA(cudaFuncSetAttribute(conv_igemm_kernel<BLOCK_N, GPT, SH, RES>, cudaFuncAttributeMaxDynamicSharedMemorySize,
                                  C::kSmemBytes));
     attr_set = true;
   }
   const int grid = p.total_tiles < sms ? p.total_tiles : sms;
-  conv_igemm_kernel<BLOCK_N, GPT, SH><<<grid, kThreads, C::kSmemBytes, st>>>(ma0, ma1, mb, mo, p);
+  conv_igemm_kernel<BLOCK_N, GPT, SH, RES><<<grid, kThreads, C::kSmemBytes, st>>>(ma0, ma1, mb, mo, mr, p);
   FD_LAUNCH_CHECK();
   return FD_OK;
 }
@@ -666,6 +688,8 @@
                                residual == nullptr && gn_stats == nullptr && Cout % 256 == 0),
              "conv_igemm: the pixel-shuffle store is for 1x1 convs with Cout %% 256 == 0, no residual / statistics");
   FD_REQUIRE(src0 && wpacked && out, "conv_igemm: null pointer");
+  FD_REQUIRE(residual == nullptr || (reinterpret_cast<uintptr_t>(residual) & 15) == 0,
+             "conv_igemm: the residual must be 16-byte aligned (it is read by TMA)");
   FD_REQUIRE(N > 0 && H > 0 && W > 0, "conv_igemm: bad geometry N=%d H=%d W=%d", N, H, W);
   FD_REQUIRE(C0 > 0 && C0 % 64 == 0 && C1 >= 0 && C1 % 64 == 0, "conv_igemm: C0=%d C1=%d must be multiples of 64", C0, C1);
   FD_REQUIRE(src1 != nullptr || C1 == 0, "conv_igemm: C1 > 0 needs src1");
@@ -784,28 +808,39 @@
     const uint32_t box[5] = {64, (uint32_t)ts.Wt, (uint32_t)ts.R, 1, 1};
     if (int e = make_tmap_bf16(&mo, out, 5, dims, str, box)) return e;
   }
+  CUtensorMap mr = mo;
+  if (residual != nullptr) {
+    FD_REQUIRE(out_mode == 0, "conv_igemm: a residual needs out_mode 0");
+    const uint64_t dims[5] = {(uint64_t)Cout, (uint64_t)p.W, (uint64_t)p.H, (uint64_t)p.N, 1};
+    const uint64_t str[4] = {(uint64_t)Cout * 2, (uint64_t)p.W * Cout * 2, (uint64_t)p.H * p.W * Cout * 2,
+                             (uint64_t)p.N * p.H * p.W * Cout * 2};
+    const uint32_t box[5] = {64, (uint32_t)ts.Wt, (uint32_t)ts.R, 1, 1};
+    if (int e = make_tmap_bf16(&mr, residual, 5, dims, str, box)) return e;
+  }
   cudaStream_t st = (cudaStream_t)stream;
   const bool stats = gn_stats != nullptr;
   if (stats) FD_REQUIRE(p.n_tiles == 1 || p.n_tiles == 2, "conv_igemm: statistics need Cout in {64,128,256,512}");
   const bool store_heavy = !stats && p.taps * (p.chunks0 + p.chunks1) <= 4;
   if (store_heavy) {
-    if (block_n == 256) return launch<256, 0, 1>(ma0, ma1, mb, mo, p, sms, st);
-    if (block_n == 128) return launch<128, 0, 1>(ma0, ma1, mb, mo, p, sms, st);
-    return launch<64, 0, 1>(ma0, ma1, mb, mo, p, sms, st);
+    if (block_n == 256) return launch<256, 0, 1>(ma0, ma1, mb, mo, mr, p, sms, st);
+    if (block_n == 128)
+      return residual ? launch<128, 0, 1, 1>(ma0, ma1, mb, mo, mr, p, sms, st) : launch<128, 0, 1>(ma0, ma1, mb, mo, mr, p, sms, st);
+    return residual ? launch<64, 0, 1, 1>(ma0, ma1, mb, mo, mr, p, sms, st) : launch<64, 0, 1>(ma0, ma1, mb, mo, mr, p, sms, st);
   }
   if (use_pair && block_n == 256) {
-    if (!stats) return launch_pair<256, 0>(ma0, ma1, mb, mo, p, sms, st);
-    return p.n_tiles == 1 ? launch_pair<256, 8>(ma0, ma1, mb, mo, p, sms, st) : launch_pair<256, 4>(ma0, ma1, mb, mo, p, sms, st);
+    if (!stats)
+      return residual ? launch_pair<256, 0, 1, 1>(ma0, ma1, mb, mo, mr, p, sms, st) : launch_pair<256, 0>(ma0, ma1, mb, mo, mr, p, sms, st);
+    return p.n_tiles == 1 ? launch_pair<256, 8>(ma0, ma1, mb, mo, mr, p, sms, st) : launch_pair<256, 4>(ma0, ma1, mb, mo, mr, p, sms, st);
   }
   if (use_pair) {
     const bool mt2 = ((long)p.N * p.tiles_w * p.tiles_h) % 4 == 0 && p.total_tiles >= 4;
-    if (mt2) return stats ? launch_pair<128, 8, 2>(ma0, ma1, mb, mo, p, sms, st) : launch_pair<128, 0, 2>(ma0, ma1, mb, mo, p, sms, st);
-    return stats ? launch_pair<128, 8>(ma0, ma1, mb, mo, p, sms, st) : launch_pair<128, 0>(ma0, ma1, mb, mo, p, sms, st);
+    if (mt2) return stats ? launch_pair<128, 8, 2>(ma0, ma1, mb, mo, mr, p, sms, st) : launch_pair<128, 0, 2>(ma0, ma1, mb, mo, mr, p, sms, st);
+    return stats ? launch_pair<128, 8>(ma0, ma1, mb, mo, mr, p, sms, st) : launch_pair<128, 0>(ma0, ma1, mb, mo, mr, p, sms, st);
   }
   if (block_n == 256) {
-    if (!stats) return launch<256, 0>(ma0, ma1, mb, mo, p, sms, st);
-    return p.n_tiles == 1 ? launch<256, 8>(ma0, ma1, mb, mo, p, sms, st) : launch<256, 4>(ma0, ma1, mb, mo, p, sms, st);
-  }
-  if (block_n == 128) return stats ? launch<128, 8>(ma0, ma1, mb, mo, p, sms, st) : launch<128, 0>(ma0, ma1, mb, mo, p, sms, st);
-  return stats ? launch<64, 8>(ma0, ma1, mb, mo, p, sms, st) : launch<64, 0>(ma0, ma1, mb, mo, p, sms, st);
-}
+    if (!stats) return launch<256, 0>(ma0, ma1, mb, mo, mr, p, sms, st);
+    return p.n_tiles == 1 ? launch<256, 8>(ma0, ma1, mb, mo, mr, p, sms, st) : launch<256, 4>(ma0, ma1, mb, mo, mr, p, sms, st);
+  }
+  if (block_n == 128) return stats ? launch<128, 8>(ma0, ma1, mb, mo, mr, p, sms, st) : launch<128, 0>(ma0, ma1, mb, mo, mr, p, sms, st);
+  return stats ? launch<64, 8>(ma0, ma1, mb, mo, mr, p, sms, st) : launch<64, 0>(ma0, ma1, mb, mo, mr, p, sms, st);
+}
diff --git a/opticalflowdiffusion_b200/csrc/fd_conv_strip.cu b/opticalflowdiffusion_b200/csrc/fd_conv_strip.cu
--- a/opticalflowdiffusion_b200/csrc/fd_conv_strip.cu
+++ b/opticalflowdiffusion_b200/csrc/fd_conv_strip.cu
@@ -14,7 +14,8 @@
 constexpr int kWBytes = 9 * kWTapBytes;
 constexpr int kThreads = 64 + kEpiThreads + 64;
 constexpr int kTail = 256 + 2 * kC * 4 + kEpiWarps * 16 * 4 + 64;
-constexpr int kSmemBytes = 1024 + kWBytes + kNS * kStripBytes + 2 * kSlabBytes + kTail;
+constexpr int kSmemBytes = 1024 + kWBytes + kNS * kStripBytes + 2 * kSlabBytes + 2 * kSlabBytes + kTail;
+static_assert(kSmemBytes <= 232448, "shared memory");
 
 __device__ __forceinline__ void utccp_128x256b(uint32_t tmem_dst, uint64_t sdesc) {
   asm volatile("tcgen05.cp.cta_group::1.128x256b [%0], %1;" ::"r"(tmem_dst), "l"(sdesc) : "memory");
@@ -75,8 +76,26 @@
   }
 };
 
-template <int GPT, class NextTile>
-__device__ __forceinline__ void strip_epilogue2(const EpiCtx& ec, NextTile next_tile) {
+struct StripTiles {
+  StripWalk walk;
+  int j = 0, n = 0, w0 = 0, ra = 0, rb = 0;
+  __device__ __forceinline__ explicit StripTiles(const StripParams& p) : walk(p) {}
+  __device__ __forceinline__ bool next(const StripParams& p, EpiTile& t) {
+    while (ra + j >= rb) {
+      if (!walk.next(p, n, w0, ra, rb)) return false;
+      j = 0;
+    }
+    t.img = n;
+    t.h0 = ra + j;
+    t.w0 = w0;
+    t.n_tile = 0;
+    ++j;
+    return true;
+  }
+};
+
+template <int GPT>
+__device__ __forceinline__ void strip_epilogue2(const EpiCtx& ec, const StripParams& p) {
   const int warp = threadIdx.x >> 5, lane = threadIdx.x & 31;
   const int ew = warp - 2;
   const int quarter = warp & 3, group = ew >> 2;
@@ -115,8 +134,27 @@
     named_bar_sync(bar_id, 128);
   };
 
+  const bool has_res = ec.residual != nullptr;
+  const uint32_t rslot = ec.r_smem + group * kSlabBytes;
+  const uint32_t rbar = ec.rfull0 + 8u * group;
+  uint32_t rphase = 0;
+  const StripWalk range(p);
+  auto res_issue = [&](int it) {
+    const int g = range.cur + it;
+    if (g >= range.end) return;
+    if ((ew & 3) == 0 && elect_one_sync()) {
+      const int col = g / p.H;
+      const int n = col / p.wblocks;
+      mbar_expect_tx(rbar, kSlabBytes);
+      tma_load_5d(rslot, ec.map_res, rbar, 0, (col - n * p.wblocks) * p.tile_w, g - col * p.H, n, 0);
+    }
+    __syncwarp();
+  };
+  if (has_res) res_issue(group);
+
+  StripTiles tiles(p);
   EpiTile tc;
-  for (int iter = 0; next_tile(iter, tc); ++iter) {
+  for (int iter = 0; tiles.next(p, tc); ++iter) {
     if ((iter & 1) != group) continue;
     const int as = group;
     const uint32_t aphase = (iter >> 1) & 1;
@@ -132,6 +170,12 @@
     if (kDiag && (ec.dbg & 8)) {
       tc_fence_before();
       mbar_arrive(ec.tempty0 + 8u * as);
+      if (has_res) {
+        mbar_wait(rbar, rphase);
+        rphase ^= 1u;
+        named_bar_sync(bar_id, 128);
+        res_issue(iter + 2);
+      }
       continue;
     }
     uint32_t acc[2][32];
@@ -141,7 +185,10 @@
     tmem_ld_wait();
     tc_fence_before();
     mbar_arrive(ec.tempty0 + 8u * as);
-    const long pix = ((long)img * ec.H + h) * ec.W + w;
+    if (has_res) {
+      mbar_wait(rbar, rphase);
+      rphase ^= 1u;
+    }
     uint32_t packed[32];
 #pragma unroll
     for (int hc = 0; hc < 2; ++hc) {
@@ -154,12 +201,15 @@
         v[j4 * 4 + 2] = __uint_as_float(acc[hc][j4 * 4 + 2]) + b4.z;
         v[j4 * 4 + 3] = __uint_as_float(acc[hc][j4 * 4 + 3]) + b4.w;
       }
-      if (ec.residual != nullptr && valid) {
-        const __nv_bfloat16* rrow = ec.residual + pix * kC + hc * 32;
+      if (has_res && valid) {
+        const uint32_t rrow = rslot + (uint32_t)row * 128u;
 #pragma unroll
         for (int q = 0; q < 4; ++q) {
-          const uint4 r4 = __ldg(reinterpret_cast<const uint4*>(rrow) + q);
-          const uint32_t rw[4] = {r4.x, r4.y, r4.z, r4.w};
+          uint32_t rw[4];
+          asm volatile("ld.shared.v4.b32 {%0, %1, %2, %3}, [%4];"
+                       : "=r"(rw[0]), "=r"(rw[1]), "=r"(rw[2]), "=r"(rw[3])
+                       : "r"(rrow + (((uint32_t)(hc * 4 + q) ^ (uint32_t)(row & 7)) << 4))
+                       : "memory");
 #pragma unroll
           for (int e = 0; e < 4; ++e) {
             const float2 f = fd_unpack_bf16(rw[e]);
@@ -187,6 +237,7 @@
     }
     if ((ew & 3) == 0 && elect_one_sync()) tma_store_wait_read<0>();
     named_bar_sync(bar_id, 128);
+    if (has_res) res_issue(iter + 2);
     const uint32_t rbase = buf + (uint32_t)row * 128u;
 #pragma unroll
     for (int q = 0; q < 8; ++q) {
@@ -210,22 +261,25 @@
 template <int GPT>
 __global__ void __launch_bounds__(kThreads, 1)
 conv3x3_strip_kernel(const __grid_constant__ CUtensorMap map_in, const __grid_constant__ CUtensorMap map_w,
-                     const __grid_constant__ CUtensorMap map_out, const StripParams p) {
+                     const __grid_constant__ CUtensorMap map_out, const __grid_constant__ CUtensorMap map_res,
+                     const StripParams p) {
   extern __shared__ uint8_t smem_raw[];
   const uint32_t base = (smem_u32(smem_raw) + 1023u) & ~1023u;
   uint8_t* gbase = smem_raw + (base - smem_u32(smem_raw));
   const uint32_t w_smem = base;
   const uint32_t s_smem = base + kWBytes;
   const uint32_t o_smem = s_smem + kNS * kStripBytes;
-  const uint32_t bar_base = o_smem + 2 * kSlabBytes;
+  const uint32_t r_smem = o_smem + 2 * kSlabBytes;
+  const uint32_t bar_base = r_smem + 2 * kSlabBytes;
   const uint32_t wfull_bar = bar_base;
   auto full_bar = [&](int s) { return bar_base + 8u * (1 + s); };
   auto empty_bar = [&](int s) { return bar_base + 8u * (1 + kNS + s); };
   auto tfull_bar = [&](int s) { return bar_base + 8u * (1 + 2 * kNS + s); };
   auto tempty_bar = [&](int s) { return bar_base + 8u * (3 + 2 * kNS + s); };
   auto xfull_bar = [&](int s) { return bar_base + 8u * (5 + 2 * kNS + s); };
+  auto rfull_bar = [&](int s) { return bar_base + 8u * (5 + 3 * kNS + s); };
   const bool fuse_in = p.in_stats != nullptr;
-  uint8_t* gtail = gbase + kWBytes + kNS * kStripBytes + 2 * kSlabBytes + 256;
+  uint8_t* gtail = gbase + kWBytes + kNS * kStripBytes + 4 * kSlabBytes + 256;
   float* s_bias = reinterpret_cast<float*>(gtail);
   float* s_stats = reinterpret_cast<float*>(gtail + 2 * kC * 4);
   uint32_t* s_tmem = reinterpret_cast<uint32_t*>(gtail + 2 * kC * 4 + kEpiWarps * 16 * 4);
@@ -235,6 +289,7 @@
     tma_prefetch_desc(&map_in);
     tma_prefetch_desc(&map_w);
     tma_prefetch_desc(&map_out);
+    if (p.residual != nullptr) tma_prefetch_desc(&map_res);
     mbar_init(wfull_bar, 1);
     for (int s = 0; s < kNS; ++s) {
       mbar_init(full_bar(s), 1);
@@ -244,6 +299,7 @@
     for (int s = 0; s < 2; ++s) {
       mbar_init(tfull_bar(s), 1);
       mbar_init(tempty_bar(s), 128);
+      mbar_init(rfull_bar(s), 1);
     }
     fence_barrier_init();
   }
@@ -511,6 +567,9 @@
     ec.map_out = &map_out;
     ec.bias = p.bias;
     ec.residual = p.residual;
+    ec.map_res = &map_res;
+    ec.r_smem = r_smem;
+    ec.rfull0 = rfull_bar(0);
     ec.gn_stats = p.gn_stats;
     ec.H = p.H; ec.W = p.W; ec.Cout = kC; ec.Wt = kTileW;
     ec.shuffle_cq = 0;
@@ -520,21 +579,7 @@
     ec.phase = -1;
     ec.head_out = nullptr; ec.head_w = nullptr; ec.head_b = nullptr; ec.head_n = 0; ec.s_head = nullptr;
     ec.head_h0 = ec.head_w0 = ec.head_pt = ec.head_pl = 0;
-    StripWalk walk(p);
-    int j = 0, n = 0, w0 = 0, ra = 0, rb = 0;
-    auto next = [&](int, EpiTile& t) {
-      while (ra + j >= rb) {
-        if (!walk.next(p, n, w0, ra, rb)) return false;
-        j = 0;
-      }
-      t.img = n;
-      t.h0 = ra + j;
-      t.w0 = w0;
-      t.n_tile = 0;
-      ++j;
-      return true;
-    };
-    strip_epilogue2<GPT>(ec, next);
+    strip_epilogue2<GPT>(ec, p);
   }
 
   tc_fence_before();
@@ -576,6 +621,8 @@
 static int strip_launch(const void* src0, int C0, const void* src1, int C1, const void* wpacked, const float* bias,
                         const void* residual, void* out, double* gn_stats, int N, int H, int W, const StripInputNorm& in,
                         cudaStream_t st) {
+  FD_REQUIRE(residual == nullptr || (reinterpret_cast<uintptr_t>(residual) & 15) == 0,
+             "conv3x3 strip: the residual must be 16-byte aligned (it is read by TMA)");
   static int sms = 0;
   if (sms == 0) {
     int dev = 0;
@@ -591,9 +638,9 @@
   p.total_rows = N * p.wblocks * H;
   p.w_kstride = cin;
   CUtensorMap mw, mo;
+  const uint64_t dO[5] = {(uint64_t)kC, (uint64_t)W, (uint64_t)H, (uint64_t)N, 1};
+  const uint64_t sO[4] = {(uint64_t)kC * 2, (uint64_t)W * kC * 2, (uint64_t)H * W * kC * 2, (uint64_t)N * H * W * kC * 2};
   {
-    const uint64_t dO[5] = {(uint64_t)kC, (uint64_t)W, (uint64_t)H, (uint64_t)N, 1};
-    const uint64_t sO[4] = {(uint64_t)kC * 2, (uint64_t)W * kC * 2, (uint64_t)H * W * kC * 2, (uint64_t)N * H * W * kC * 2};
     const uint32_t box_out[5] = {64, (uint32_t)p.tile_w, 1, 1, 1};
     if (int e = make_tmap_bf16(&mo, out, 5, dO, sO, box_out)) return e;
     const uint64_t K = (uint64_t)9 * cin;
@@ -631,9 +678,14 @@
     p.w_k0 = pass * 64;
     p.bias = last ? bias : nullptr;
     p.residual = static_cast<const __nv_bfloat16*>(pass > 0 ? out : residual);
+    CUtensorMap mr = mo;
+    if (p.residual != nullptr && p.residual != out) {
+      const uint32_t box_out[5] = {64, (uint32_t)p.tile_w, 1, 1, 1};
+      if (int e = make_tmap_bf16(&mr, p.residual, 5, dO, sO, box_out)) return e;
+    }
     p.gn_stats = last ? gn_stats : nullptr;
-    if (p.gn_stats != nullptr) conv3x3_strip_kernel<8><<<grid, kThreads, kSmemBytes, st>>>(mi, mw, mo, p);
-    else conv3x3_strip_kernel<0><<<grid, kThreads, kSmemBytes, st>>>(mi, mw, mo, p);
+    if (p.gn_stats != nullptr) conv3x3_strip_kernel<8><<<grid, kThreads, kSmemBytes, st>>>(mi, mw, mo, mr, p);
+    else conv3x3_strip_kernel<0><<<grid, kThreads, kSmemBytes, st>>>(mi, mw, mo, mr, p);
     FD_LAUNCH_CHECK();
   }
   return FD_OK;
```

Result: faster. 9.462, median of 6 (+2.7%).
